# hwwang55/GraphGAN

Hardware: AMD Instinct MI355X
Metric: sampled_edges_per_sec (higher is better)
Workload: dtype f32

## Files before the change

### graphgan_amd/csrc/gg_api.hip

```cpp
#include <stdarg.h>
#include <stdlib.h>
#include <string.h>
#include <sys/stat.h>
#include <unistd.h>

#include <algorithm>
#include <atomic>
#include <thread>

#include "gg_internal.h"

namespace gg {

thread_local std::string g_last_error;

int fail(gg_ctx *ctx, int code, const char *fmt, ...) {
    char buf[1024];
    va_list ap;
    va_start(ap, fmt);
    vsnprintf(buf, sizeof(buf), fmt, ap);
    va_end(ap);
    g_last_error = buf;
    if (ctx) ctx->err = buf;
    return code;
// ... 199 lines not shown
    ctx->w_nslots = n_slots;
    ctx->w_uniform = (!n_walks && uniform_walks >= 0) ? uniform_walks : -1;
    ctx->w_args = {for_d, seed, stream};
    ctx->g_paths_valid = false;
    if (ctx->g_slots_ready) {
        GG_HIP(ctx, hipStreamWaitEvent(ctx->stream, ctx->ev_slots_done, 0));
        ctx->g_slots_ready = false;
        ctx->g_slots_unused++;
    }
    if (n_slots == 0) {
        ctx->walk_stream = ctx->stream;
        return GG_OK;
    }
    return launch_and_join(ctx, n_slots, total, for_d, seed, stream, stride, !defer_join);
}

int gg::walk_finalize(gg_ctx *ctx, bool *retried) {
    if (retried) *retried = false;
    if (ctx->w_nslots == 0) {
        GG_HIP(ctx, hipStreamSynchronize(ctx->stream));
        return GG_OK;
    }
    const int64_t total = ctx->w_total;
    unsigned long long *c = ctx->h_pin;
    constexpr int CW = gg_ctx::CTR_WORDS;
    GG_HIP(ctx, hipMemcpyAsync(c, ctx->dev_ctr, sizeof(unsigned long long) * 2 * CW, hipMemcpyDeviceToHost, ctx->stream));
    GG_HIP(ctx, hipStreamSynchronize(ctx->stream));
    harvest_timings(ctx);
    for (int attempt = 0; c[3] == 2ull || (c[2] != 0ull && ctx->t_lazy); ++attempt) {
        GG_CHECK(ctx, attempt < 16, GG_EHIP, "walk: the launch was voided %d times in a row", attempt);
        if (c[2] != 0ull && ctx->t_lazy) {
            int rebuilt = 0;
            int rc = lazy_fallback_rebuild(ctx, &rebuilt);
            if (rc == GG_ECAPACITY) rc = lazy_rebuild_whole(ctx);
            if (rc != GG_OK) return rc;
            if (ctx->tree_max_depth + 3 > ctx->w_stride) {
                ctx->w_stride = ctx->tree_max_depth + 3;
                GG_HIP(ctx, ctx->w_paths.reserve(sizeof(int32_t) * ((size_t)total * ctx->w_stride + 1)));
            }
        } else {
            ctx->walk_force_sized = true;
        }
        ctx->ctr.walk_reruns += 1;
        generator_changed(ctx);
        int rc = launch_and_join(ctx, ctx->w_nslots, total, ctx->w_args.for_d, ctx->w_args.seed, ctx->w_args.stream, ctx->w_stride);
        ctx->walk_force_sized = false;
        if (rc != GG_OK) return rc;
        GG_HIP(ctx, hipMemcpyAsync(c, ctx->dev_ctr, sizeof(unsigned long long) * 2 * CW, hipMemcpyDeviceToHost, ctx->stream));
        GG_HIP(ctx, hipStreamSynchronize(ctx->stream));
        if (retried) *retried = true;
    }
    const int n_half = ctx->w_split ? 2 : 1;
    if (n_half == 2)
        for (int i = 8; i < CW; ++i) c[i] += c[CW + i];
    {
        int64_t *prof = ctx->alive_prof[ctx->w_args.for_d ? 1 : 0];
        const int run = ctx->w_levels_run;
        for (int i = 0; i < 64; ++i) prof[i] = i < run ? (int64_t)c[8 + i] : -1;
        if (run > 0 && run < 64 && ctx->w_fin_follows) prof[run] = (int64_t)c[7];
        if (ctx->w_net && c[7] > 2048ull && ctx->lv_levels_learned < ctx->tree_max_depth + 2) ctx->lv_levels_learned += 1;
    }
    unsigned long long hops = c[0], reads = c[1], rows = c[5];
    unsigned long long gathers = 0, nodes = 0;
    for (int i = 0; i < 64; ++i) { hops += c[264 + i]; reads += c[328 + i]; rows += c[200 + i]; gathers += c[520 + i]; nodes += c[584 + i]; }
    ctx->ctr.es_gathers += (int64_t)gathers;
    ctx->ctr.es_nodes += (int64_t)nodes;
    ctx->ctr.hops += (int64_t)hops;
    ctx->ctr.nbr_reads += (int64_t)reads;
    ctx->ctr.rows_scored += (int64_t)rows;
    ctx->ctr.walks += total;
    if (total && ctx->walk_timed) {
        float ms = 0.f;
        GG_HIP(ctx, hipEventElapsedTime(&ms, ctx->ev0, ctx->ev1));
        ctx->ctr.last_kernel_ms = ms;
        ctx->ctr.walk_kernel_ms += ms;
        ctx->ctr.walk_launches += 1;
        for (int i = 0; i < ctx->lv_ev_used; ++i) {
            float lms = 0.f;
            for (int k = 0; k < n_half; ++k) {
                float e = 0.f;
                GG_HIP(ctx, hipEventElapsedTime(&e, ctx->lv_ev[4 * i + 2 * k], ctx->lv_ev[4 * i + 2 * k + 1]));
                lms += e;
            }
            ctx->ctr.score_kernel_ms += lms;
            ctx->ctr.score_launches += n_half;
            ctx->ctr.score_chunks += (int64_t)(c[136 + i] >> 32);
            if (getenv("GG_WALK_DEBUG"))
                fprintf(stderr, "[walk] for_d=%d level %d alive %llu score chunks %llu prefix chunks %llu big %llu small %llu rows %llu score %.1f us\n", ctx->w_args.for_d, i,
                        c[8 + i], c[136 + i] >> 32, c[136 + i] & 0xffffffffull, c[72 + i] & 0xffffffffull, c[72 + i] >> 32, c[456 + i], lms * 1e3);
        }
        if (ctx->lv_ev_used) {
            ctx->ctr.score_rows += (int64_t)(rows - c[5]);
            unsigned long long dists = 0;
            for (int i = 0; i < 64; ++i) dists += c[392 + i];
            ctx->ctr.score_dists += (int64_t)dists;
            ctx->ctr.score_gathers += (int64_t)gathers;
            ctx->ctr.score_nodes += (int64_t)nodes;
        }
    }
    if (c[3] || c[6]) generator_changed(ctx);
    if (c[3]) return fail(ctx, GG_ECAPACITY, "walk: a path needed more than stride=%d entries", ctx->w_stride);
    if (c[6]) return fail(ctx, GG_EINVAL, "walk: non-finite generator scores (a softmax had total weight 0, or the generator's tables hold a non-finite value)");
    return GG_OK;
}

int gg::walk_resident(gg_ctx *ctx, const int32_t *slots, const int32_t *n_walks, int32_t uniform_walks, int32_t n_slots,
                      int32_t for_d, uint64_t seed, uint32_t stream, int32_t stride) {
    int rc = walk_launch_async(ctx, slots, n_walks, uniform_walks, n_slots, for_d, seed, stream, stride);
    if (rc != GG_OK) return rc;
    return walk_finalize(ctx, nullptr);
}

extern "C" {

int gg_abi_version(void) { return GG_ABI_VERSION; }

const char *gg_last_error(const gg_ctx *ctx) { return ctx ? ctx->err.c_str() : g_last_error.c_str(); }

int gg_create(int32_t n_node, int32_t n_emb, const float *emb_gen, const float *emb_dis, const gg_config *cfg,
              gg_ctx **out) {
    if (!out) return fail(nullptr, GG_EINVAL, "gg_create: out is NULL");
    *out = nullptr;
    if (n_node <= 0 || n_emb <= 0 || n_emb > 512 || !emb_gen || !emb_dis || !cfg)
        return fail(nullptr, GG_EINVAL, "gg_create: bad argument (n_node=%d n_emb=%d)", n_node, n_emb);
    int ndev = 0;
    hipError_t e = hipGetDeviceCount(&ndev);
    if (e != hipSuccess || ndev <= 0)
        return fail(nullptr, GG_EHIP, "gg_create: no HIP device (%s); this engine has no CPU fallback",
                    e == hipSuccess ? "count = 0" : hipGetErrorString(e));
    if (cfg->device < 0 || cfg->device >= ndev) return fail(nullptr, GG_EINVAL, "gg_create: device %d of %d", cfg->device, ndev);
    hipDeviceProp_t prop;
    GG_HIP(nullptr, hipGetDeviceProperties(&prop, cfg->device));
    if (strncmp(prop.gcnArchName, "gfx950", 6) != 0)
        return fail(nullptr, GG_EHIP, "gg_create: device %d is %s; kernels are built for gfx950 only", cfg->device, prop.gcnArchName);
    GG_HIP(nullptr, hipSetDevice(cfg->device));

    gg_ctx *ctx = new gg_ctx();
    ctx->n_node = n_node;
    ctx->n_emb = n_emb;
    ctx->ld = (n_emb + 3) / 4 * 4;
    ctx->cfg = *cfg;
    ctx->device = cfg->device;
    ctx->n_cus = prop.multiProcessorCount > 0 ? prop.multiProcessorCount : 256;
    if (const char *lv = getenv("GG_WALK_LEVELS")) ctx->walk_levels = atoi(lv);
    if (const char *pe = getenv("GG_PROFILE_EVERY")) ctx->profile_every = std::max(0, atoi(pe));
    if (const char *fw = getenv("GG_COMM_FAKE_WORLD")) ctx->fake_world = atoi(fw);
    if (const char *ow = getenv("GG_COMM_OWNER")) ctx->owner_exchange = atoi(ow);
    if (const char *bf = getenv("GG_COMM_BF16")) ctx->comm_bf16 = atoi(bf) != 0;
    if (const char *om = getenv("GG_COMM_OWNER_MIN")) ctx->owner_min_bound = atoll(om);
    if (const char *dt = getenv("GG_DETERMINISTIC")) ctx->deterministic = atoi(dt) != 0;
    if (const char *nc = getenv("GG_NO_DIST_CACHE")) ctx->dc_enabled = atoi(nc) == 0;
    if (const char *ft = getenv("GG_FIN_THRESHOLD")) ctx->fin_threshold = std::max(0, atoi(ft));
    if (const char *st = getenv("GG_STAGE_T")) ctx->sg_threshold = std::max(0, atoi(st));
    if (const char *ws = getenv("GG_WALK_SPLIT")) ctx->split_enabled = atoi(ws) != 0;
    if (const char *em = getenv("GG_ES_MODE")) ctx->es_mode = std::min(2, std::max(0, atoi(em)));
    if (const char *er = getenv("GG_ES_RATIO")) ctx->es_ratio_num = std::max(1, atoi(er));
    if (const char *eh = getenv("GG_ES_HUB")) ctx->es_hub = std::max(0, atoi(eh));
    if (const char *wm = getenv("GG_WALK_SPLIT_MIN")) ctx->split_min_walks = std::max(512, atoi(wm));
    for (auto &m : ctx->alive_prof) for (auto &v : m) v = -1;
    if (const char *dr = getenv("GG_COMM_DENSE_RATIO")) ctx->dense_exchange_ratio = (float)atof(dr);
#define GG_TRY(call)                        \
    do {                                    \
        int rc__ = (call);                  \
        if (rc__ != GG_OK) {                \
            g_last_error = ctx->err;        \
            gg_destroy(ctx);                \
            return rc__;                    \
        }                                   \
    } while (0)
    auto body = [&]() -> int {
        GG_HIP(ctx, hipStreamCreateWithFlags(&ctx->stream, hipStreamNonBlocking));
        {
            int lo = 0, hi = 0;
            const char *wp = getenv("GG_WALK_PRIORITY");
            if (wp && atoi(wp) != 0 && hipDeviceGetStreamPriorityRange(&lo, &hi) == hipSuccess && hi != lo)
                GG_HIP(ctx, hipStreamCreateWithPriority(&ctx->stream2, hipStreamNonBlocking, atoi(wp) > 0 ? hi : lo));
            else
                GG_HIP(ctx, hipStreamCreateWithFlags(&ctx->stream2, hipStreamNonBlocking));
        }
        GG_HIP(ctx, hipStreamCreateWithFlags(&ctx->stream3, hipStreamNonBlocking));
        GG_HIP(ctx, hipEventCreateWithFlags(&ctx->ev_fork, hipEventDisableTiming));
        GG_HIP(ctx, hipEventCreateWithFlags(&ctx->ev_join, hipEventDisableTiming));
        GG_HIP(ctx, hipEventCreateWithFlags(&ctx->ev_score[0], hipEventDisableTiming));
        GG_HIP(ctx, hipEventCreateWithFlags(&ctx->ev_score[1], hipEventDisableTiming));
        ctx->walk_stream = ctx->stream;
        GG_HIP(ctx, hipEventCreate(&ctx->ev0));
        GG_HIP(ctx, hipEventCreate(&ctx->ev1));
        GG_HIP(ctx, hipEventCreateWithFlags(&ctx->ev_walk_done, hipEventDisableTiming));
        GG_HIP(ctx, hipEventCreateWithFlags(&ctx->ev_gen_pass, hipEventDisableTiming));
        GG_HIP(ctx, hipEventCreateWithFlags(&ctx->ev_main_mark, hipEventDisableTiming));
        GG_HIP(ctx, hipHostMalloc((void **)&ctx->h_pin, sizeof(unsigned long long) * gg_ctx::PIN_WORDS, hipHostMallocDefault));
        memset(ctx->h_pin, 0, sizeof(unsigned long long) * gg_ctx::PIN_WORDS);
        const size_t tb = sizeof(float) * (size_t)n_node * ctx->ld, vb = sizeof(float) * (size_t)n_node;
        for (int m = 0; m < 2; ++m) {
            Model &M = ctx->model[m];
            GG_HIP(ctx, hipMalloc((void **)&M.E, tb));
            GG_HIP(ctx, hipMalloc((void **)&M.b, vb));
            GG_HIP(ctx, hipMemset(M.b, 0, vb));
            if (cfg->optimizer != GG_OPT_SGD) {
                GG_HIP(ctx, hipMalloc((void **)&M.mE, tb));
                GG_HIP(ctx, hipMalloc((void **)&M.vE, tb));
                GG_HIP(ctx, hipMalloc((void **)&M.mb, vb));
                GG_HIP(ctx, hipMalloc((void **)&M.vb, vb));
                GG_HIP(ctx, hipMemset(M.mE, 0, tb));
                GG_HIP(ctx, hipMemset(M.vE, 0, tb));
                GG_HIP(ctx, hipMemset(M.mb, 0, vb));
                GG_HIP(ctx, hipMemset(M.vb, 0, vb));
            }
            M.b1p = cfg->adam_beta1;
            M.b2p = cfg->adam_beta2;
            M.lr = m == 0 ? cfg->lr_gen : cfg->lr_dis;
            M.lambda = m == 0 ? cfg->lambda_gen : cfg->lambda_dis;
            int rc = upload_table(ctx, M.E, m == 0 ? emb_gen : emb_dis);
            if (rc != GG_OK) return rc;
        }
        GG_HIP(ctx, hipMalloc((void **)&ctx->gradE, tb));
        GG_HIP(ctx, hipMalloc((void **)&ctx->gradb, vb));
        GG_HIP(ctx, hipMemset(ctx->gradE, 0, tb));
        ctx->grad_elems_padded = (size_t)n_node * ctx->ld;
        GG_HIP(ctx, hipMemset(ctx->gradb, 0, vb));
        GG_HIP(ctx, hipMalloc((void **)&ctx->touched, sizeof(int32_t) * n_node));
        GG_HIP(ctx, hipMalloc((void **)&ctx->touched_list, sizeof(int32_t) * n_node));
        GG_HIP(ctx, hipMalloc((void **)&ctx->touched_cnt, sizeof(int32_t) * 4));
        GG_HIP(ctx, hipMemset(ctx->touched, 0, sizeof(int32_t) * n_node));
        GG_HIP(ctx, hipMemset(ctx->touched_cnt, 0, sizeof(int32_t) * 4));
        GG_HIP(ctx, hipMalloc((void **)&ctx->dev_ctr, sizeof(unsigned long long) * gg_ctx::PIN_WORDS));
        GG_HIP(ctx, hipMemset(ctx->dev_ctr, 0, sizeof(unsigned long long) * gg_ctx::PIN_WORDS));
        GG_HIP(ctx, ctx->table_bad.reserve(sizeof(unsigned long long) * 2));
        for (int m = 0; m < 2; ++m) {
            int rc = rescan_table_finite(ctx, m);
            if (rc != GG_OK) return rc;
        }
        GG_HIP(ctx, hipDeviceSynchronize());
        return GG_OK;
    };
    GG_TRY(body());
#undef GG_TRY
    *out = ctx;
    return GG_OK;
}

int gg_destroy(gg_ctx *ctx) {
    if (!ctx) return GG_OK;
    (void)hipSetDevice(ctx->device);
    if (ctx->stream) (void)hipStreamSynchronize(ctx->stream);
    if (ctx->stream2) (void)hipStreamSynchronize(ctx->stream2);
    comm_destroy(ctx);
    for (int m = 0; m < 2; ++m) {
        Model &M = ctx->model[m];
        float *ps[] = {M.E, M.b, M.mE, M.vE, M.mb, M.vb};
        for (float *p : ps)
            if (p) (void)hipFree(p);
    }
    void *ps[] = {ctx->gradE, ctx->gradb, ctx->touched, ctx->touched_list, ctx->touched_cnt, ctx->g_rowptr, ctx->g_col, ctx->dev_ctr,
                  ctx->es, ctx->es_stamp, ctx->g_rev};
    for (void *p : ps)
        if (p) (void)hipFree(p);
    free_trees(ctx);
    DevBuf *bufs[] = {&ctx->w_slots_m[0], &ctx->w_slots_m[1], &ctx->w_ptr_m[0], &ctx->w_ptr_m[1], &ctx->w_samples, &ctx->w_paths, &ctx->w_len, &ctx->w_status,
                      &ctx->w_first, &ctx->w_abort, &ctx->w_scratch, &ctx->d_center, &ctx->d_neighbor, &ctx->d_label, &ctx->d_cnt,
                      &ctx->d_ptr, &ctx->g_node1, &ctx->g_node2, &ctx->g_reward, &ctx->g_cnt, &ctx->g_ptr, &ctx->scan_tmp,
                      &ctx->step_u, &ctx->step_v, &ctx->step_x, &ctx->sg_cnt, &ctx->sg_off, &ctx->sg_slot, &ctx->sg_list, &ctx->sg_rows, &ctx->sg_bias, &ctx->sg_tot, &ctx->sg_key, &ctx->touched_ptr, &ctx->x_cnt, &ctx->x_send_ids, &ctx->x_send_rows,
                      &ctx->x_recv_ids, &ctx->x_recv_rows, &ctx->x_nglob, &ctx->x_own, &ctx->st_item, &ctx->st_item2, &ctx->st_cur, &ctx->st_prev, &ctx->st_len,
                      &ctx->st_alive, &ctx->st_rank, &ctx->bfs_key, &ctx->bfs_bm, &ctx->bfs_misc, &ctx->bfs_sparse, &ctx->bfs_rowptr32, &ctx->lv_pfx, &ctx->dc_keys, &ctx->dc_vals, &ctx->dc_words, &ctx->lv_beg, &ctx->lv_k, &ctx->lv_chunks, &ctx->lv_coff, &ctx->lv_scores, &ctx->lv_chunk_owner, &ctx->lv_prefix, &ctx->lv_big, &ctx->lv_fe, &ctx->fin_list, &ctx->table_bad, &ctx->sgp_cnt, &ctx->sgp_off, &ctx->sgp_slot, &ctx->sgp_list, &ctx->sgp_tot, &ctx->sgp_key, &ctx->sgp_scan, &ctx->sgp_hub, &ctx->sg_hub, &ctx->hub_acc,
                      &ctx->q3_store, &ctx->q3s_off, &ctx->ep_center, &ctx->ep_neighbor, &ctx->ep_label, &ctx->ep_node1, &ctx->ep_node2, &ctx->ep_reward, &ctx->topk_adj,
                      &ctx->gs_es, &ctx->gs_cpre, &ctx->pt_starts, &ctx->pt_paths, &ctx->pt_len, &ctx->pt_cnt, &ctx->pt_ptr, &ctx->pt_noise, &ctx->pt_sample};
    for (DevBuf *b : bufs) b->release();
    for (hipEvent_t e : ctx->lv_ev)
        if (e) (void)hipEventDestroy(e);
    for (auto &tr : ctx->tm_ev)
        for (hipEvent_t e : tr)
            if (e) (void)hipEventDestroy(e);
    for (hipEvent_t e : ctx->pt_ev)
        if (e) (void)hipEventDestroy(e);
    if (ctx->h_pin) (void)hipHostFree(ctx->h_pin);
    for (hipEvent_t e : {ctx->ev_walk_done, ctx->ev_slots_done, ctx->ev_gen_pass, ctx->ev_main_mark, ctx->ev_fork, ctx->ev_join, ctx->ev_score[0], ctx->ev_score[1]})
        if (e) (void)hipEventDestroy(e);
    if (ctx->stream3) {
        (void)hipStreamSynchronize(ctx->stream3);
        (void)hipStreamDestroy(ctx->stream3);
    }
    if (ctx->stream2) {
        (void)hipStreamSynchronize(ctx->stream2);
        (void)hipStreamDestroy(ctx->stream2);
    }
    if (ctx->ev0) (void)hipEventDestroy(ctx->ev0);
    if (ctx->ev1) (void)hipEventDestroy(ctx->ev1);
    if (ctx->stream) (void)hipStreamDestroy(ctx->stream);
    delete ctx;
    return GG_OK;
}

int gg_set_graph_csr(gg_ctx *ctx, const int64_t *rowptr, const int32_t *col) {
    if (!ctx) return fail(nullptr, GG_EINVAL, "ctx is NULL");
    GG_CHECK(ctx, rowptr && rowptr[0] == 0, GG_EINVAL, "gg_set_graph_csr: rowptr[0] must be 0");
    discard_begun_walk(ctx);
    const int n = ctx->n_node;
    const int64_t nnz = rowptr[n];
    GG_CHECK(ctx, nnz >= 0 && (col || nnz == 0), GG_EINVAL, "gg_set_graph_csr: col is NULL");
    for (int v = 0; v < n; ++v) GG_CHECK(ctx, rowptr[v + 1] >= rowptr[v], GG_EINVAL, "gg_set_graph_csr: rowptr not monotone at %d", v);
    for (int64_t e = 0; e < nnz; ++e) GG_CHECK(ctx, col[e] >= 0 && col[e] < n, GG_EINVAL, "gg_set_graph_csr: col[%lld]=%d out of range", (long long)e, col[e]);
    GG_HIP(ctx, hipSetDevice(ctx->device));
    (void)hipDeviceSynchronize();
    for (void *p : {(void *)ctx->g_rowptr, (void *)ctx->g_col, (void *)ctx->es, (void *)ctx->es_stamp, (void *)ctx->g_rev})
        if (p) (void)hipFree(p);
    ctx->g_rowptr = nullptr;
// ... 652 lines not shown
```

### graphgan_amd/csrc/gg_internal.h

```cpp
#pragma once
#include <hip/hip_runtime.h>
#include <stdint.h>
#include <stdio.h>
#include <string>
#include <vector>

#include "../../include/graphgan_hip.h"

namespace gg {

struct DevBuf {
    void *p = nullptr;
    size_t bytes = 0;
    hipError_t reserve(size_t need) {
        if (need <= bytes) return hipSuccess;
        if (p) {
            (void)hipDeviceSynchronize();
            (void)hipFree(p);
        }
        p = nullptr;
        bytes = 0;
        size_t want = need + need / 4 + 256;
        hipError_t e = hipMalloc(&p, want);
        if (e == hipSuccess) bytes = want;
// ... 17 lines not shown
};

}

struct gg_ctx {
    int32_t n_node = 0, n_emb = 0, ld = 0;
    gg_config cfg{};
    int device = 0;
    hipStream_t stream = nullptr;
    hipEvent_t ev0 = nullptr, ev1 = nullptr;
    hipStream_t stream2 = nullptr;
    hipStream_t walk_stream = nullptr;
    hipEvent_t ev_walk_done = nullptr;
    hipEvent_t ev_gen_pass = nullptr;
    hipEvent_t ev_main_mark = nullptr;
    bool gen_pass_recorded = false;
    bool gen_dirty = false;
    hipEvent_t lv_ev[256] = {};
    hipStream_t stream3 = nullptr;
    hipEvent_t ev_fork = nullptr, ev_join = nullptr, ev_score[2] = {nullptr, nullptr};
    bool split_enabled = false;
    int64_t split_min_walks = 32768;
    bool w_split = false;
    gg::DevBuf fin_list;
    gg::DevBuf table_bad;
    int lv_ev_used = 0;
    gg::Model model[2];

    float *gradE = nullptr, *gradb = nullptr;
    int32_t *touched = nullptr;
    int32_t *touched_list = nullptr;
    int32_t *touched_cnt = nullptr;

    int64_t *g_rowptr = nullptr;
    int32_t *g_col = nullptr;
    int64_t g_nnz = 0;
    uint64_t g_hash = 0;
    std::vector<int64_t> h_rowptr;
    std::vector<int32_t> h_col;
    float *es = nullptr;
    long long *es_stamp = nullptr;
    int32_t *g_rev = nullptr;
    long long es_tick = 256;
    long long es_valid_from = 256;
    int32_t es_mode = 1;
    int32_t es_ratio_num = 2;
    int32_t es_hub = 0;

    int32_t n_tree_roots = 0, tree_max_depth = 0, tree_max_list = 0;
    int64_t tree_nodes = 0;
    int64_t t_cap_nodes = 0, t_cap_roots = 0, t_cap_q3 = 0;
    int64_t tree_entries = 0;
    int32_t *t_root = nullptr;
    int32_t *t_order = nullptr;
    int32_t *t_cstart = nullptr;
    int32_t *t_edge = nullptr;
    bool t_edge_valid = false;
    int64_t *t_base = nullptr;
    uint32_t *t_q3 = nullptr;
    int64_t *t_q3off = nullptr;
    std::vector<int32_t> h_troot;
    std::vector<int64_t> h_tbase, h_q3off;
    std::vector<int32_t> h_comp_size;

    int32_t tree_mode = -1;
    int64_t lz_cap = 0;
    bool t_lazy = false;
    bool lz_force_whole = false;
    int32_t lz_min_level = 0x7fffffff;
    uint32_t lz_stamp = 0;
    gg::DevBuf lz_info, lz_pair, lz_rank, lz_bm, lz_cursor, lz_flag, lz_limit, lz_expect, lz_list, lz_scratch, lz_fb_scratch;
    int64_t arena_next = 0, arena_end = 0;
    int64_t lz_fallback_roots = 0, lz_fallback_rounds = 0, lz_resolved = 0;
    bool g_multi = true;
    int32_t g_max_deg = 0;

    gg::DevBuf w_slots_m[2], w_ptr_m[2];
    std::vector<int32_t> h_slots_m[2];
    std::vector<int64_t> h_ptr_m[2], h_ptr_new;
    int w_mode = 0;
    int64_t alive_prof[2][64];
    int64_t fin_threshold = 0;
    int w_levels_run = 0;
    bool w_fin_follows = false;
    bool w_net = false;
    const gg::DevBuf &w_slots_buf() const { return w_slots_m[w_mode]; }
    const gg::DevBuf &w_ptr_buf() const { return w_ptr_m[w_mode]; }
    gg::DevBuf w_samples, w_paths, w_len, w_status, w_first, w_abort, w_scratch;
    gg::DevBuf st_cur, st_prev, st_len, st_alive, st_rank, st_item, st_item2, lv_beg, lv_k, lv_chunks, lv_coff, lv_scores, lv_chunk_owner, lv_prefix, lv_big, lv_fe;
    gg::DevBuf lv_pfx, dc_keys, dc_vals, dc_words;
    size_t dc_size = 0;
    int32_t dc_request = 0;
    bool dc_valid = false;
    bool dc_enabled = true;
    int64_t lv_cap_total = 0;
    int32_t lv_levels_learned = 0;
    int64_t lv_cap_chunks = 0;
    bool walk_force_sized = false;
    bool walk_used_speculation = false;
    int32_t walk_levels = 64;
    int64_t w_total = 0;
    int32_t w_stride = 0, w_nslots = 0;
    int32_t w_uniform = -1;
    struct { int32_t for_d; uint64_t seed; uint32_t stream; } w_args{};

    static constexpr int CTR_WORDS = 720;
    static constexpr int PIN_WORDS = 2048;
    static constexpr int H_TOTAL = 1960;
    static constexpr int H_ROWS = 1940;
    unsigned long long *h_pin = nullptr;
    int32_t profile_every = 1;
    int64_t walk_call_index = 0;
    bool walk_timed = false;
    bool profile_solo = true;
    struct PendingTiming { int kind; int64_t units; int slot; bool has_rows; };
    hipEvent_t tm_ev[8][3] = {};
    std::vector<PendingTiming> tm_pending;
    int64_t pass_call_index[2] = {0, 0};
    int tm_cur = -1;

    gg::DevBuf d_center, d_neighbor, d_label, d_cnt, d_ptr;
    int64_t d_rows = 0;
    gg::DevBuf g_node1, g_node2, g_reward, g_cnt, g_ptr;
    int64_t g_pairs = 0;
    bool g_paths_valid = false;
    bool g_begun = false;
    struct { int32_t n_slots = 0, n_sample = 0; uint64_t seed = 0; uint32_t stream = 0; } g_begun_args;
    gg::DevBuf touched_ptr;
    gg::DevBuf bfs_key, bfs_bm, bfs_misc, bfs_sparse, bfs_rowptr32;
    bool bfs_rowptr32_valid = false;
    gg::DevBuf q3_store, q3s_off;
    int64_t q3_words = 0;
    bool q3_store_ready = false;
    gg::DevBuf ep_center, ep_neighbor, ep_label, ep_node1, ep_node2, ep_reward;
    int64_t ep_rows = 0, ep_pairs = 0;
    std::vector<int32_t> ep_slots;
    bool in_epoch_add = false;
    int n_cus = 256;
    gg::DevBuf scan_tmp, step_u, step_v, step_x;
    gg::DevBuf sg_cnt, sg_off, sg_slot, sg_list, sg_rows, sg_bias, sg_tot, sg_key;
    bool g_pairs_filled = false;
    bool sg_cnt_dirty = false;
    gg::DevBuf sgp_cnt, sgp_off, sgp_slot, sgp_list, sgp_tot, sgp_key, sgp_scan, sgp_hub;
    gg::DevBuf sg_hub, hub_acc;
    int64_t hub_cap = 0;
    hipEvent_t ev_slots_done = nullptr;
    bool g_slots_ready = false;
    bool sgp_cnt_clean = false;
    int g_slots_unused = 0;
    int64_t g_slots_walks = 0;
    int32_t g_slots_stride = 0;
    int32_t *sg_cnt_active = nullptr;
    bool sg_active = false;
    int sg_threshold = 64;

    unsigned long long *dev_ctr = nullptr;
    gg_counters ctr{};

    void *comm = nullptr;
    bool comm_rsag = true;
    size_t grad_elems_padded = 0;
    int64_t d_rows_max = 0, g_pairs_max = 0;
    int64_t step_bound = 0;
    int64_t comm_steps_sparse = 0, comm_steps_dense = 0, comm_bytes_sent = 0;
    int32_t rank = 0, world = 1;
    bool deterministic = true;
    float dense_exchange_ratio = 1.5f;
    int32_t fake_world = 0;
    gg::DevBuf x_cnt, x_send_ids, x_send_rows, x_recv_ids, x_recv_rows;
    gg::DevBuf x_nglob;
    gg::DevBuf x_own;
    int32_t owner_exchange = 1;
    bool comm_bf16 = false;
    int64_t owner_min_bound = 4096;
    int64_t comm_steps_owner = 0;

    gg::DevBuf topk_adj;
    bool topk_adj_valid = false;

    gg::DevBuf gs_es, gs_cpre;
    int64_t gs_chunks = 0;
    bool gs_es_valid = false, gs_cpre_valid = false;

    gg::DevBuf pt_starts, pt_paths, pt_len, pt_cnt, pt_ptr, pt_noise, pt_sample;
    bool pt_noise_set = false;
    uint64_t pt_noise_total = 0;
    int32_t pt_sample_n = 0, pt_sample_stride = 1;
    hipEvent_t pt_ev[4] = {};
    bool ep_d_open = false;

    std::string err;
};

namespace gg {

extern thread_local std::string g_last_error;

int fail(gg_ctx *ctx, int code, const char *fmt, ...);

#define GG_HIP(ctx, call)                                                                      \
    do {                                                                                       \
        hipError_t e__ = (call);                                                               \
        if (e__ != hipSuccess)                                                                 \
            return gg::fail(ctx, GG_EHIP, "%s:%d %s -> %s", __FILE__, __LINE__, #call,         \
                            hipGetErrorString(e__));                                           \
    } while (0)

#define GG_CHECK(ctx, cond, code, ...)                        \
    do {                                                      \
        if (!(cond)) return gg::fail(ctx, code, __VA_ARGS__); \
    } while (0)

int device_exclusive_scan(gg_ctx *ctx, const int32_t *cnt, int64_t *ptr, int64_t n);
int ensure_g_pairs(gg_ctx *ctx);
int device_compact_flags(gg_ctx *ctx, const int32_t *flag, int64_t n, int32_t *list, int64_t *total_out);
int device_segment_rows(gg_ctx *ctx, const int32_t *cnt, int64_t n, int T, int32_t *off, int4 *list, int64_t *totals, hipStream_t stream = nullptr,
                        DevBuf *scratch = nullptr);

int alloc_trees(gg_ctx *ctx, const int32_t *roots, int32_t n_roots, const int64_t *node_counts, const int64_t *root_children, int64_t extra_nodes = 0);
bool lazy_build_wanted(const gg_ctx *ctx);
int lazy_rebuild_whole(gg_ctx *ctx);
int lazy_fallback_rebuild(gg_ctx *ctx, int *n_out);
void component_sizes(int n, const int64_t *rowptr, const int32_t *col, std::vector<int32_t> &comp_size);
int32_t host_bfs_order(const int64_t *rowptr, const int32_t *col, int32_t root, int32_t *order, int32_t *cstart,
                       std::vector<uint32_t> &stamp, uint32_t &epoch, int32_t *depth_out, int32_t *max_children_out);
void order_to_lists(int32_t n, int32_t C, const int32_t *order, const int32_t *cstart, const uint32_t *q3, int32_t *off, int32_t *nbr);
int32_t lists_to_order(int32_t n, int32_t root, const int32_t *off, const int32_t *nbr, int32_t *order, int32_t *cstart,
                       uint32_t *q3, int32_t q3_words, int32_t *depth_out, int32_t *max_children_out);

int walk_launch_async(gg_ctx *ctx, const int32_t *slots, const int32_t *n_walks, int32_t uniform_walks, int32_t n_slots,
                      int32_t for_d, uint64_t seed, uint32_t stream, int32_t stride, bool side_stream = false, bool defer_join = false);
void discard_begun_walk(gg_ctx *ctx);
int walk_finalize(gg_ctx *ctx, bool *retried);
int timing_slot(gg_ctx *ctx);
int check_exchange_flag(gg_ctx *ctx);
void harvest_timings(gg_ctx *ctx);
int derive_tree_edges(gg_ctx *ctx);
int compute_reverse_edges(gg_ctx *ctx);
int rescan_table_finite(gg_ctx *ctx, int which);
int enqueue_path_slots(gg_ctx *ctx);
void generator_changed(gg_ctx *ctx);
int walk_resident(gg_ctx *ctx, const int32_t *slots, const int32_t *n_walks, int32_t uniform_walks, int32_t n_slots,
                  int32_t for_d, uint64_t seed, uint32_t stream, int32_t stride);
int launch_walk_sample(gg_ctx *ctx, int32_t n_slots, int64_t total_walks, int for_d, uint64_t seed, uint32_t stream,
                       int32_t stride);
int run_step(gg_ctx *ctx, int which, const int32_t *d_u, const int32_t *d_v, const float *d_x, int32_t n);
int comm_allreduce_grads(gg_ctx *ctx);
int comm_allreduce_flags(gg_ctx *ctx);
int comm_allreduce_i64(gg_ctx *ctx, int64_t *buf, size_t count);
int comm_allreduce_max_i64(gg_ctx *ctx, int64_t *buf, size_t count);
size_t comm_dense_bytes(const gg_ctx *ctx);
int exchange_count_max(gg_ctx *ctx, int64_t local, int64_t *max_out);
int comm_allgather(gg_ctx *ctx, const void *send, void *recv, size_t count, int elem_bytes);
bool comm_has_p2p(const gg_ctx *ctx);
int comm_exchange_v(gg_ctx *ctx, const float *send, const int64_t *send_off, const int64_t *send_cnt, float *recv, const int64_t *recv_off,
                    const int64_t *recv_cnt);
void comm_destroy(gg_ctx *ctx);

static inline int cdiv(int64_t a, int64_t b) { return (int)((a + b - 1) / b); }

}
```

### graphgan_amd/csrc/prepare.hip

```cpp
#include <algorithm>

#include <cstring>

#include "gg_internal.h"

namespace gg {

constexpr int SCAN_THREADS = 256;
constexpr int SCAN_ITEMS = 8;
constexpr int SCAN_TILE = SCAN_THREADS * SCAN_ITEMS;

__device__ __forceinline__ int64_t block_excl_scan(int64_t v, int64_t *total, int64_t *sh ) {
    const int lane = threadIdx.x & 63, wv = threadIdx.x >> 6;
    int64_t inc = v;
#pragma unroll
    for (int off = 1; off < 64; off <<= 1) {
        const int64_t o = __shfl_up(inc, off, 64);
        if (lane >= off) inc += o;
    }
    if (lane == 63) sh[wv] = inc;
    __syncthreads();
    int64_t base = 0, tot = 0;
#pragma unroll
    for (int i = 0; i < SCAN_THREADS / 64; ++i) {
        if (i < wv) base += sh[i];
        tot += sh[i];
    }
    __syncthreads();
    *total = tot;
    return base + inc - v;
}

__global__ __launch_bounds__(SCAN_THREADS) void scan_tile_sums(const int32_t *cnt, int64_t n, int64_t *tile_sum) {
    __shared__ int64_t sh[SCAN_THREADS / 64];
    const int64_t base = (int64_t)blockIdx.x * SCAN_TILE + (int64_t)threadIdx.x * SCAN_ITEMS;
    int64_t s = 0;
#pragma unroll
    for (int i = 0; i < SCAN_ITEMS; ++i)
        if (base + i < n) s += cnt[base + i];
    int64_t tot;
    (void)block_excl_scan(s, &tot, sh);
    if (threadIdx.x == 0) tile_sum[blockIdx.x] = tot;
}

__global__ __launch_bounds__(SCAN_THREADS) void scan_tile_offsets(int64_t *tile_sum, int64_t n_tiles, int64_t *total_out) {
    __shared__ int64_t sh[SCAN_THREADS / 64];
    int64_t carry = 0;
    for (int64_t t0 = 0; t0 < n_tiles; t0 += SCAN_THREADS) {
        const int64_t i = t0 + threadIdx.x;
        const int64_t v = i < n_tiles ? tile_sum[i] : 0;
        int64_t tot;
        const int64_t ex = block_excl_scan(v, &tot, sh);
        if (i < n_tiles) tile_sum[i] = carry + ex;
        carry += tot;
    }
    if (threadIdx.x == 0) *total_out = carry;
}

__global__ __launch_bounds__(SCAN_THREADS) void scan_tile_offsets2(int64_t *tile_sum_a, int64_t *tile_sum_b, int64_t n_tiles, int64_t *total_a, int64_t *total_b) {
    __shared__ int64_t sh[SCAN_THREADS / 64];
    int64_t *const tile_sum = blockIdx.x == 0 ? tile_sum_a : tile_sum_b;
    int64_t carry = 0;
    for (int64_t t0 = 0; t0 < n_tiles; t0 += SCAN_THREADS) {
        const int64_t i = t0 + threadIdx.x;
        const int64_t v = i < n_tiles ? tile_sum[i] : 0;
        int64_t tot;
        const int64_t ex = block_excl_scan(v, &tot, sh);
        if (i < n_tiles) tile_sum[i] = carry + ex;
        carry += tot;
    }
    if (threadIdx.x == 0) *(blockIdx.x == 0 ? total_a : total_b) = carry;
}

__global__ __launch_bounds__(SCAN_THREADS) void scan_apply(const int32_t *cnt, int64_t n, const int64_t *tile_off, int64_t *ptr) {
    __shared__ int64_t sh[SCAN_THREADS / 64];
    const int64_t base = (int64_t)blockIdx.x * SCAN_TILE + (int64_t)threadIdx.x * SCAN_ITEMS;
    int64_t v[SCAN_ITEMS], s = 0;
#pragma unroll
    for (int i = 0; i < SCAN_ITEMS; ++i) {
        v[i] = base + i < n ? cnt[base + i] : 0;
        s += v[i];
    }
    int64_t tot;
    int64_t run = tile_off[blockIdx.x] + block_excl_scan(s, &tot, sh);
#pragma unroll
    for (int i = 0; i < SCAN_ITEMS; ++i) {
        if (base + i < n) ptr[base + i] = run;
        run += v[i];
    }
}

int device_exclusive_scan(gg_ctx *ctx, const int32_t *cnt, int64_t *ptr, int64_t n) {
    const int64_t tiles = (n + SCAN_TILE - 1) / SCAN_TILE;
    GG_HIP(ctx, ctx->scan_tmp.reserve(sizeof(int64_t) * (tiles + 2)));
    int64_t *ts = ctx->scan_tmp.as<int64_t>();
    if (n == 0) {
        GG_HIP(ctx, hipMemsetAsync(ptr, 0, sizeof(int64_t), ctx->stream));
        return GG_OK;
    }
    hipLaunchKernelGGL(scan_tile_sums, dim3((unsigned)tiles), dim3(SCAN_THREADS), 0, ctx->stream, cnt, n, ts);
    hipLaunchKernelGGL(scan_tile_offsets, dim3(1), dim3(SCAN_THREADS), 0, ctx->stream, ts, tiles, ptr + n);
    hipLaunchKernelGGL(scan_apply, dim3((unsigned)tiles), dim3(SCAN_THREADS), 0, ctx->stream, cnt, n, ts, ptr);
    GG_HIP(ctx, hipGetLastError());
    return GG_OK;
}

__global__ __launch_bounds__(SCAN_THREADS) void flag_tile_sums(const int32_t *flag, int64_t n, int64_t *tile_sum) {
    __shared__ int64_t sh[SCAN_THREADS / 64];
    const int64_t base = (int64_t)blockIdx.x * SCAN_TILE + (int64_t)threadIdx.x * SCAN_ITEMS;
    int64_t s = 0;
#pragma unroll
    for (int i = 0; i < SCAN_ITEMS; ++i)
        if (base + i < n) s += flag[base + i] > 0 ? 1 : 0;
    int64_t tot;
    (void)block_excl_scan(s, &tot, sh);
    if (threadIdx.x == 0) tile_sum[blockIdx.x] = tot;
}

__global__ __launch_bounds__(SCAN_THREADS) void flag_compact(const int32_t *flag, int64_t n, const int64_t *tile_off, int32_t *list) {
    __shared__ int64_t sh[SCAN_THREADS / 64];
    const int64_t base = (int64_t)blockIdx.x * SCAN_TILE + (int64_t)threadIdx.x * SCAN_ITEMS;
    bool v[SCAN_ITEMS];
    int64_t s = 0;
#pragma unroll
    for (int i = 0; i < SCAN_ITEMS; ++i) {
        v[i] = base + i < n && flag[base + i] > 0;
        s += v[i] ? 1 : 0;
    }
    int64_t tot;
    int64_t run = tile_off[blockIdx.x] + block_excl_scan(s, &tot, sh);
#pragma unroll
    for (int i = 0; i < SCAN_ITEMS; ++i)
        if (v[i]) list[run++] = (int32_t)(base + i);
}

int device_compact_flags(gg_ctx *ctx, const int32_t *flag, int64_t n, int32_t *list, int64_t *total_out) {
    const int64_t tiles = (n + SCAN_TILE - 1) / SCAN_TILE;
    GG_HIP(ctx, ctx->scan_tmp.reserve(sizeof(int64_t) * (tiles + 2)));
    int64_t *ts = ctx->scan_tmp.as<int64_t>();
    if (n == 0) {
        GG_HIP(ctx, hipMemsetAsync(total_out, 0, sizeof(int64_t), ctx->stream));
        return GG_OK;
    }
    hipLaunchKernelGGL(flag_tile_sums, dim3((unsigned)tiles), dim3(SCAN_THREADS), 0, ctx->stream, flag, n, ts);
    hipLaunchKernelGGL(scan_tile_offsets, dim3(1), dim3(SCAN_THREADS), 0, ctx->stream, ts, tiles, total_out);
    hipLaunchKernelGGL(flag_compact, dim3((unsigned)tiles), dim3(SCAN_THREADS), 0, ctx->stream, flag, n, ts, list);
    GG_HIP(ctx, hipGetLastError());
    return GG_OK;
}

__global__ __launch_bounds__(SCAN_THREADS) void seg_tile_sums(const int32_t *cnt, int64_t n, int T, int64_t *tile_rows, int64_t *tile_occ) {
    __shared__ int64_t sh[SCAN_THREADS / 64];
    const int64_t base = (int64_t)blockIdx.x * SCAN_TILE + (int64_t)threadIdx.x * SCAN_ITEMS;
    int64_t rows = 0, occ = 0;
#pragma unroll
    for (int i = 0; i < SCAN_ITEMS; ++i)
        if (base + i < n) {
            const int c = cnt[base + i];
            if (c > 0 && c <= T) { rows += 1; occ += c; }
        }
    int64_t tot;
    (void)block_excl_scan(rows, &tot, sh);
    if (threadIdx.x == 0) tile_rows[blockIdx.x] = tot;
    (void)block_excl_scan(occ, &tot, sh);
    if (threadIdx.x == 0) tile_occ[blockIdx.x] = tot;
}

__global__ __launch_bounds__(SCAN_THREADS) void seg_apply(const int32_t *cnt, int64_t n, int T, const int64_t *tile_rows, const int64_t *tile_occ,
                                                          int32_t *off, int4 *list) {
    __shared__ int64_t sh[SCAN_THREADS / 64];
    const int64_t base = (int64_t)blockIdx.x * SCAN_TILE + (int64_t)threadIdx.x * SCAN_ITEMS;
    int c[SCAN_ITEMS];
    int64_t rows = 0, occ = 0;
#pragma unroll
    for (int i = 0; i < SCAN_ITEMS; ++i) {
        const int v = base + i < n ? cnt[base + i] : 0;
        c[i] = (v > 0 && v <= T) ? v : 0;
        rows += c[i] ? 1 : 0;
        occ += c[i];
    }
    int64_t tot;
    int64_t rrun = tile_rows[blockIdx.x] + block_excl_scan(rows, &tot, sh);
    int64_t orun = tile_occ[blockIdx.x] + block_excl_scan(occ, &tot, sh);
#pragma unroll
    for (int i = 0; i < SCAN_ITEMS; ++i)
        if (c[i]) {
            list[rrun++] = make_int4((int32_t)(base + i), (int32_t)orun, c[i], 0);
            off[base + i] = (int32_t)orun;
            orun += c[i];
        }
}

int device_segment_rows(gg_ctx *ctx, const int32_t *cnt, int64_t n, int T, int32_t *off, int4 *list, int64_t *totals, hipStream_t stream, DevBuf *scratch) {
    const int64_t tiles = (n + SCAN_TILE - 1) / SCAN_TILE;
    if (!scratch) scratch = &ctx->scan_tmp;
    if (!stream) stream = ctx->stream;
    GG_HIP(ctx, scratch->reserve(sizeof(int64_t) * (2 * tiles + 4)));
    int64_t *tr = scratch->as<int64_t>(), *to = tr + tiles + 1;
    hipLaunchKernelGGL(seg_tile_sums, dim3((unsigned)tiles), dim3(SCAN_THREADS), 0, stream, cnt, n, T, tr, to);
    hipLaunchKernelGGL(scan_tile_offsets2, dim3(2), dim3(SCAN_THREADS), 0, stream, tr, to, tiles, totals, totals + 1);
    hipLaunchKernelGGL(seg_apply, dim3((unsigned)tiles), dim3(SCAN_THREADS), 0, stream, cnt, n, T, tr, to, off, list);
    GG_HIP(ctx, hipGetLastError());
    return GG_OK;
}

__global__ void pair_count_kernel(const int32_t *path_len, int64_t n_walks, int window, int32_t *cnt, const unsigned long long *flag) {
    const int64_t w = (int64_t)blockIdx.x * blockDim.x + threadIdx.x;
    if (w >= n_walks) return;
    if (*flag == 2ull) { cnt[w] = 0; return; }
    const int L = path_len[w] - 1;
    int c = 0;
    for (int i = 0; i < L; ++i) {
        const int lo = max(i - window, 0), hi = min(i + window + 1, L);
        c += hi - lo - 1;
    }
    cnt[w] = L > 0 ? c : 0;
}

__global__ void pair_fill_kernel(const int32_t *paths, const int32_t *path_len, int stride, int64_t n_walks, int window,
                                 const int64_t *ptr, int32_t *node1, int32_t *node2, const unsigned long long *flag) {
    const int64_t w = (int64_t)blockIdx.x * blockDim.x + threadIdx.x;
    if (w >= n_walks || *flag == 2ull) return;
    const int L = path_len[w] - 1;
    const int32_t *p = paths + w * (int64_t)stride;
    int64_t o = ptr[w];
    for (int i = 0; i < L; ++i) {
        const int lo = max(i - window, 0), hi = min(i + window + 1, L);
        const int c = p[i];
        for (int j = lo; j < hi; ++j) {
            if (j == i) continue;
            node1[o] = c;
            node2[o] = p[j];
            ++o;
        }
    }
}

__global__ __launch_bounds__(256) void pair_reward_kernel(const float *E, const float *bias, int ld, const int32_t *u,
                                                          const int32_t *v, int64_t n_host, const int64_t *n_dev, float *out) {
    const int64_t n = n_dev ? *n_dev : n_host;
    const int t = threadIdx.x & 15;
    const int64_t g0 = ((int64_t)blockIdx.x * blockDim.x + threadIdx.x) >> 4;
    const int64_t ng = ((int64_t)gridDim.x * blockDim.x) >> 4;
    const int nchunk = ld >> 2;
    for (int64_t p = g0; p < n; p += ng) {
        const int a = u[p], b = v[p];
        const float4 *ra = (const float4 *)(E + (int64_t)a * ld);
        const float4 *rb = (const float4 *)(E + (int64_t)b * ld);
        float acc = 0.f;
        for (int c = t; c < nchunk; c += 16) {
            const float4 x = ra[c], y = rb[c];
            acc = __builtin_fmaf(x.x, y.x, acc);
            acc = __builtin_fmaf(x.y, y.y, acc);
            acc = __builtin_fmaf(x.z, y.z, acc);
            acc = __builtin_fmaf(x.w, y.w, acc);
        }
        acc += __shfl_xor(acc, 8, 64);
        acc += __shfl_xor(acc, 4, 64);
        acc += __shfl_xor(acc, 2, 64);
        acc += __shfl_xor(acc, 1, 64);
        if (t == 0) {
            float s = acc + bias[b];
            s = fminf(fmaxf(s, -10.0f), 10.0f);
            out[p] = logf(1.0f + expf(s));
        }
    }
}

template <int NCH>
__global__ __launch_bounds__(256) void path_reward_kernel(const float *E, const float *bias, int ld, const int32_t *paths,
                                                          const int32_t *path_len, int stride, int64_t n_walks, int window,
                                                          const int64_t *ptr, float *out, const unsigned long long *flag) {
    const int t = threadIdx.x & 15;
    const int64_t w = ((int64_t)blockIdx.x * blockDim.x + threadIdx.x) >> 4;
    if (w >= n_walks || *flag == 2ull) return;
    const int L = path_len[w] - 1;
    if (L <= 1) return;
    const int32_t *p = paths + w * (int64_t)stride;
    const int nchunk = ld >> 2;
    const int64_t pi0 = ptr[w];
    float4 R[3][NCH];
    float bv[3];
    bool have[3];
    auto fetch = [&](int pos, float4 (&row)[NCH], float &b, bool &ok) {
        ok = pos >= 0 && pos < L;
        const int nd = ok ? p[pos] : 0;
        b = ok ? bias[nd] : 0.f;
        const float4 *r = (const float4 *)(E + (int64_t)nd * ld);
#pragma unroll
        for (int i = 0; i < NCH; ++i) {
            const int c = t + 16 * i;
            row[i] = (ok && c < nchunk) ? r[c] : make_float4(0.f, 0.f, 0.f, 0.f);
        }
    };
    fetch(0, R[0], bv[0], have[0]);
    fetch(1, R[1], bv[1], have[1]);
    fetch(2, R[2], bv[2], have[2]);
    auto n_pairs_of = [&](int i) { return min(i, window) + min(L - 1 - i, window); };
    int base = 0;
    for (int c = 0; c < L; ++c) {
        float4 Rn[NCH];
        float nb;
        bool nh;
        fetch(c + 3, Rn, nb, nh);
        const int back_c = min(c, window);
        int base_d = base + n_pairs_of(c);
        float myval = 0.f;
        int myidx = -1;
#pragma unroll
        for (int d = 1; d <= 2; ++d) {
            if (d <= window && have[d]) {
                float acc = 0.f;
#pragma unroll
                for (int i = 0; i < NCH; ++i) {
                    acc = __builtin_fmaf(R[0][i].x, R[d][i].x, acc);
                    acc = __builtin_fmaf(R[0][i].y, R[d][i].y, acc);
                    acc = __builtin_fmaf(R[0][i].z, R[d][i].z, acc);
                    acc = __builtin_fmaf(R[0][i].w, R[d][i].w, acc);
                }
                acc += __shfl_xor(acc, 8, 64);
                acc += __shfl_xor(acc, 4, 64);
                acc += __shfl_xor(acc, 2, 64);
                acc += __shfl_xor(acc, 1, 64);
                if (t == 2 * d - 2) { myval = acc + bv[d]; myidx = base + back_c + (d - 1); }
                if (t == 2 * d - 1) { myval = acc + bv[0]; myidx = base_d + (c - max(c + d - window, 0)); }
            }
            base_d += n_pairs_of(c + d);
        }
        if (myidx >= 0) {
            const float sc = fminf(fmaxf(myval, -10.0f), 10.0f);
            out[pi0 + myidx] = logf(1.0f + expf(sc));
        }
        base += n_pairs_of(c);
#pragma unroll
        for (int i = 0; i < NCH; ++i) { R[0][i] = R[1][i]; R[1][i] = R[2][i]; R[2][i] = Rn[i]; }
        have[0] = have[1]; have[1] = have[2]; have[2] = nh;
        bv[0] = bv[1]; bv[1] = bv[2]; bv[2] = nb;
    }
}

__global__ __launch_bounds__(256) void edge_dot_f64_kernel(const float *E, int ld, const int32_t *u, const int32_t *v, int64_t n, double *out) {
    const int t = threadIdx.x & 15;
    const int64_t g0 = ((int64_t)blockIdx.x * blockDim.x + threadIdx.x) >> 4, ng = ((int64_t)gridDim.x * blockDim.x) >> 4;
    for (int64_t p = g0; p < n; p += ng) {
        const float *ra = E + (int64_t)u[p] * ld, *rb = E + (int64_t)v[p] * ld;
        double acc = 0.0;
        for (int k = t; k < ld; k += 16) acc = fma((double)ra[k], (double)rb[k], acc);
        acc += __shfl_xor(acc, 8, 64);
        acc += __shfl_xor(acc, 4, 64);
        acc += __shfl_xor(acc, 2, 64);
        acc += __shfl_xor(acc, 1, 64);
        if (t == 0) out[p] = acc;
    }
}
// ... 315 lines not shown
```

### graphgan_amd/csrc/steps.hip

```cpp
#include <stdlib.h>

#include <algorithm>
#include <cmath>
#include <vector>

#include "gg_internal.h"

namespace gg {

struct HubAcc {
    unsigned long long *acc;
    int64_t cap;
    float scale;
};
__device__ __forceinline__ unsigned long long *hub_row(const HubAcc &h, int slot, int ld) {
    const int64_t k = -3 - (int64_t)slot;
    return (slot <= -3 && k < h.cap) ? h.acc + k * (ld + 1) : nullptr;
}
__device__ __forceinline__ void hub_add(unsigned long long *p, float x, float scale) {
    atomicAdd(p, (unsigned long long)__float2ll_rn(x * scale));
}

struct StepArgs {
    float *E, *b;
    float *gE, *gb;
    int32_t *touched, *touched_list, *touched_cnt;
    int ld, track;
    const int32_t *u, *v;
    const float *x;
    int n;
    float lambda, inv_n;
    const int64_t *n_glob;
    int is_d;
    int ppg;
    unsigned long long *prof;
    const int32_t *slot_v, *slot_u;
    float *stage, *stage_b;
    HubAcc hub;
};

__global__ __launch_bounds__(256) void pair_occ_count_kernel(const int32_t *u, const int32_t *v, int n, int ppg, int32_t *cnt,
                                                             int32_t *slot_v, int32_t *slot_u) {
    const int p = blockIdx.x * blockDim.x + threadIdx.x;
    if (p >= n) return;
    slot_v[p] = atomicAdd(&cnt[v[p]], 1);
    const bool run_end = p == n - 1 || (p + 1) % ppg == 0 || u[p + 1] != u[p];
    slot_u[p] = run_end ? atomicAdd(&cnt[u[p]], 1) : -2;
}

__global__ __launch_bounds__(256) void pair_occ_slot_kernel(const int32_t *u, const int32_t *v, int n, const int32_t *cnt, const int32_t *off,
                                                            int T, int32_t *slot_v, int32_t *slot_u, int32_t *key) {
    const int p = blockIdx.x * blockDim.x + threadIdx.x;
    if (p >= n) return;
    const int iv = v[p], iu = u[p];
    const int sv = cnt[iv] <= T ? off[iv] + slot_v[p] : -3 - off[iv];
    slot_v[p] = sv;
    if (sv >= 0) key[sv] = 2 * p + 1;
    if (slot_u[p] != -2) {
        const int su = cnt[iu] <= T ? off[iu] + slot_u[p] : -3 - off[iu];
        slot_u[p] = su;
        if (su >= 0) key[su] = 2 * p;
    }
}

constexpr int PAIRS_PER_GROUP = 16;

template <int NF, bool STAGED>
__global__ __launch_bounds__(256) void pair_grad_kernel(const StepArgs a) {
    const int t = threadIdx.x & 15;
    const int g = (blockIdx.x * blockDim.x + threadIdx.x) >> 4;
    const int p0 = g * a.ppg;
    if (p0 >= a.n) return;
    const int p1 = min(p0 + a.ppg, a.n);
    const int nchunk = a.ld >> 2;
    const float inv_n = a.n_glob ? 1.0f / (float)(*a.n_glob) : a.inv_n;
    float accu[NF];
#pragma unroll
    for (int i = 0; i < NF; ++i) accu[i] = 0.f;
    int run_u = a.u[p0];
    auto flush_u = [&](int q) {
        const int sl = STAGED ? a.slot_u[q] : -1;
        if (STAGED && sl >= 0) {
            float *g = a.stage + (int64_t)sl * a.ld;
#pragma unroll
            for (int i = 0; i < NF; ++i) {
                const int f = t + 16 * i;
                if (f < a.ld) g[f] = accu[i];
            }
            if (t == 0) a.stage_b[sl] = 0.f;
            return;
        }
        float *gu = a.gE + (int64_t)run_u * a.ld;
#pragma unroll
        for (int i = 0; i < NF; ++i) {
            const int f = t + 16 * i;
            if (f < a.ld) atomicAdd(gu + f, accu[i]);
        }
        if (t == 0 && a.track) a.touched[run_u] = 1;
    };
    for (int p = p0; p < p1; ++p) {
        const int iu = a.u[p], iv = a.v[p];
        if (iu != run_u) {
            flush_u(p - 1);
#pragma unroll
            for (int i = 0; i < NF; ++i) accu[i] = 0.f;
            run_u = iu;
        }
        const float4 *ru = (const float4 *)(a.E + (int64_t)iu * a.ld);
        const float4 *rv = (const float4 *)(a.E + (int64_t)iv * a.ld);
        float acc = 0.f;
        for (int c = t; c < nchunk; c += 16) {
            const float4 x = ru[c], y = rv[c];
            acc = __builtin_fmaf(x.x, y.x, acc);
            acc = __builtin_fmaf(x.y, y.y, acc);
            acc = __builtin_fmaf(x.z, y.z, acc);
            acc = __builtin_fmaf(x.w, y.w, acc);
        }
        acc += __shfl_xor(acc, 8, 64);
        acc += __shfl_xor(acc, 4, 64);
        acc += __shfl_xor(acc, 2, 64);
        acc += __shfl_xor(acc, 1, 64);
        const float bv = a.b[iv];
        const float s = acc + bv;
        const float sg = 1.0f / (1.0f + expf(-s));
        float ds;
        if (a.is_d) {
            ds = sg - a.x[p];
        } else {
            const bool inside = (sg >= 1e-5f) && (sg <= 1.0f);
            ds = inside ? -(a.x[p] * inv_n) * (1.0f - sg) : 0.0f;
        }
        const float *fu = (const float *)ru, *fv = (const float *)rv;
        const int slv = STAGED ? a.slot_v[p] : -1;
        const bool st = STAGED && slv >= 0;
        float *gv = st ? a.stage + (int64_t)slv * a.ld : a.gE + (int64_t)iv * a.ld;
#pragma unroll
        for (int i = 0; i < NF; ++i) {
            const int f = t + 16 * i;
            if (f < a.ld) {
                const float x = fu[f], y = fv[f];
                accu[i] += ds * y + a.lambda * x;
                const float gval = ds * x + a.lambda * y;
                if (st) gv[f] = gval;
                else atomicAdd(gv + f, gval);
            }
        }
        if (t == 0) {
            const float gbv = a.is_d ? ds + a.lambda * bv : ds;
            if (st) {
                a.stage_b[slv] = gbv;
            } else {
                atomicAdd(a.gb + iv, gbv);
                if (a.track) a.touched[iv] = 1;
            }
        }
    }
    flush_u(p1 - 1);
}

template <int NF, bool STAGED>
__global__ __launch_bounds__(256) void pair_grad16_kernel(const StepArgs a) {
    const int t = threadIdx.x & 15;
    const int64_t g = ((int64_t)blockIdx.x * blockDim.x + threadIdx.x) >> 4;
    const int64_t p0 = g * 16;
    if (p0 >= a.n) return;
    const int np = (int)min((int64_t)16, (int64_t)a.n - p0);
    const float inv_n = a.n_glob ? 1.0f / (float)(*a.n_glob) : a.inv_n;
    const bool mine = t < np;
    const int myu = mine ? a.u[p0 + t] : 0, myv = mine ? a.v[p0 + t] : 0;
    const float myx = mine ? a.x[p0 + t] : 0.f;
    const int my_sv = (STAGED && mine) ? a.slot_v[p0 + t] : -1;
    const int my_su = (STAGED && mine) ? a.slot_u[p0 + t] : -1;
    const float mybv = a.b[myv];
    const int nextu = __shfl(myu, (t + 1) & 15, 16);
    const bool my_end = mine && (t == np - 1 || nextu != myu);
    auto fetch = [&](int j, float (&ru)[NF], float (&rv)[NF]) {
        const int jj = j < np ? j : 0;
        const float *su = a.E + (int64_t)__shfl(myu, jj, 16) * a.ld, *sv = a.E + (int64_t)__shfl(myv, jj, 16) * a.ld;
#pragma unroll
        for (int i = 0; i < NF; ++i) {
            const int f = t + 16 * i;
            const int fc = f < a.ld ? f : a.ld - 1;
            ru[i] = su[fc];
            rv[i] = sv[fc];
        }
    };
    float U[3][NF], V[3][NF], accu[NF];
#pragma unroll
    for (int i = 0; i < NF; ++i) accu[i] = 0.f;
    fetch(0, U[0], V[0]);
    fetch(1, U[1], V[1]);
#pragma unroll 1
    for (int j0 = 0; j0 < np; j0 += 3) {
#pragma unroll
        for (int r = 0; r < 3; ++r) {
            const int j = j0 + r;
            if (j >= np) break;
            fetch(j + 2, U[(r + 2) % 3], V[(r + 2) % 3]);
            float acc = 0.f;
#pragma unroll
            for (int i = 0; i < NF; ++i) {
                const bool in = t + 16 * i < a.ld;
                const float x = in ? U[r][i] : 0.f, y = in ? V[r][i] : 0.f;
                U[r][i] = x; V[r][i] = y;
                acc = __builtin_fmaf(x, y, acc);
            }
            acc += __shfl_xor(acc, 8, 64);
            acc += __shfl_xor(acc, 4, 64);
            acc += __shfl_xor(acc, 2, 64);
            acc += __shfl_xor(acc, 1, 64);
            const float bv = __shfl(mybv, j, 16), xj = __shfl(myx, j, 16);
            const float s = acc + bv;
            const float sg = 1.0f / (1.0f + expf(-s));
            float ds;
            if (a.is_d) {
                ds = sg - xj;
            } else {
                const bool inside = (sg >= 1e-5f) && (sg <= 1.0f);
                ds = inside ? -(xj * inv_n) * (1.0f - sg) : 0.0f;
            }
            const int iv = __shfl(myv, j, 16), iu = __shfl(myu, j, 16);
            const int slv = __shfl(my_sv, j, 16), slu = __shfl(my_su, j, 16);
            const bool st = STAGED && slv >= 0;
            unsigned long long *hv = STAGED && !st ? hub_row(a.hub, slv, a.ld) : nullptr;
            float *gv = st ? a.stage + (int64_t)slv * a.ld : a.gE + (int64_t)iv * a.ld;
#pragma unroll
            for (int i = 0; i < NF; ++i) {
                const int f = t + 16 * i;
                if (f < a.ld) {
                    accu[i] += ds * V[r][i] + a.lambda * U[r][i];
                    const float gval = ds * U[r][i] + a.lambda * V[r][i];
                    if (st) gv[f] = gval;
                    else if (STAGED && hv) hub_add(hv + f, gval, a.hub.scale);
                    else atomicAdd(gv + f, gval);
                }
            }
            if (t == 0) {
                const float gbv = a.is_d ? ds + a.lambda * bv : ds;
                if (st) {
                    a.stage_b[slv] = gbv;
                } else {
                    if (STAGED && hv) hub_add(hv + a.ld, gbv, a.hub.scale);
                    else atomicAdd(a.gb + iv, gbv);
                    if (a.track) a.touched[iv] = 1;
                }
            }
            if (__shfl((int)my_end, j, 16)) {
                if (STAGED && slu >= 0) {
                    float *gu = a.stage + (int64_t)slu * a.ld;
#pragma unroll
                    for (int i = 0; i < NF; ++i) {
                        const int f = t + 16 * i;
                        if (f < a.ld) gu[f] = accu[i];
                    }
                    if (t == 0) a.stage_b[slu] = 0.f;
                } else {
                    float *gu = a.gE + (int64_t)iu * a.ld;
                    unsigned long long *hu = STAGED ? hub_row(a.hub, slu, a.ld) : nullptr;
#pragma unroll
                    for (int i = 0; i < NF; ++i) {
                        const int f = t + 16 * i;
                        if (f < a.ld) {
                            if (STAGED && hu) hub_add(hu + f, accu[i], a.hub.scale);
                            else atomicAdd(gu + f, accu[i]);
                        }
                    }
                    if (t == 0 && a.track) a.touched[iu] = 1;
                }
#pragma unroll
                for (int i = 0; i < NF; ++i) accu[i] = 0.f;
            }
        }
    }
}

struct PathArgs {
    float *E, *b, *gE, *gb;
    int32_t *touched, *touched_list, *touched_cnt;
    int ld, track, window;
    const int32_t *paths, *path_len;
    int stride;
    const int64_t *pair_ptr;
    const float *reward;
    int64_t n_walks;
    float lambda, inv_n;
    const int64_t *n_glob;
    const int32_t *slot;
    float *stage, *stage_b;
    HubAcc hub;
};

__global__ __launch_bounds__(256) void path_count_kernel(const int32_t *paths, const int32_t *path_len, int stride, int64_t n_walks,
                                                         int32_t *cnt, int32_t *slot, const unsigned long long *flag) {
    const int64_t idx = (int64_t)blockIdx.x * blockDim.x + threadIdx.x;
    const int64_t w = idx / stride;
    if (w >= n_walks || (flag && *flag == 2ull)) return;
    const int c = (int)(idx - w * stride), L = path_len[w] - 1;
    if (L <= 1 || c >= L) return;
    slot[idx] = atomicAdd(&cnt[paths[idx]], 1);
}

__global__ __launch_bounds__(256) void path_slot_kernel(const int32_t *paths, const int32_t *path_len, int stride, int64_t n_walks,
                                                        const int32_t *cnt, const int32_t *off, int T, int32_t *slot, int32_t *key, const unsigned long long *flag) {
    const int64_t idx = (int64_t)blockIdx.x * blockDim.x + threadIdx.x;
    const int64_t w = idx / stride;
    if (w >= n_walks || (flag && *flag == 2ull)) return;
    const int c = (int)(idx - w * stride), L = path_len[w] - 1;
    if (L <= 1 || c >= L) return;
    const int nd = paths[idx];
    const int sl = cnt[nd] <= T ? off[nd] + slot[idx] : -3 - off[nd];
    slot[idx] = sl;
    if (sl >= 0) key[sl] = (int32_t)idx;
}

template <int NF, bool STAGED, bool SHORT>
__global__ __launch_bounds__(256) __attribute__((amdgpu_waves_per_eu(NF <= 8 ? 3 : 1, 4))) void path_grad_kernel(const PathArgs a) {
    const int t = threadIdx.x & 15;
    const int64_t w = ((int64_t)blockIdx.x * blockDim.x + threadIdx.x) >> 4;
    if (w >= a.n_walks) return;
    const int L = a.path_len[w] - 1;
    if (L <= 1) return;
    const float inv_n = a.n_glob ? 1.0f / (float)(*a.n_glob) : a.inv_n;
    const int32_t *p = a.paths + w * (int64_t)a.stride;
    int64_t pi = a.pair_ptr[w];
    const int32_t *const wslot = STAGED ? a.slot + w * (int64_t)a.stride : nullptr;
    const int myid = (t < L) ? p[t] : -1;
    const int myslot = (STAGED && t < L) ? wslot[t] : -1;
    const int64_t pi0 = pi;
    const int n_pairs = (int)(a.pair_ptr[w + 1] - pi0);
    float rwl[4];
#pragma unroll
    for (int q = 0; q < 4; ++q) rwl[q] = (16 * q + t < n_pairs) ? a.reward[pi0 + 16 * q + t] : 0.f;
    auto id_at = [&](int pos) -> int {
        if (SHORT) {
            const int v = __shfl(myid, pos & 15, 16);
            return (pos >= 0 && pos < L) ? v : -1;
        }
        return (pos >= 0 && pos < L) ? (pos < 16 ? __shfl(myid, pos, 16) : p[pos]) : -1;
    };
    auto slot_at = [&](int pos) -> int {
        if (!STAGED) return -1;
        if (SHORT) {
            const int v = __shfl(myslot, pos & 15, 16);
            return (pos >= 0 && pos < L) ? v : -1;
        }
        return (pos >= 0 && pos < L) ? (pos < 16 ? __shfl(myslot, pos, 16) : wslot[pos]) : -1;
    };
    auto reward_at = [&](int k, int64_t pidx) -> float {
        const float v0 = __shfl(rwl[0], k & 15, 16), v1 = __shfl(rwl[1], k & 15, 16);
        const float v2 = __shfl(rwl[2], k & 15, 16), v3 = __shfl(rwl[3], k & 15, 16);
        const float v = k < 16 ? v0 : (k < 32 ? v1 : (k < 48 ? v2 : v3));
        if (SHORT) return v;
        return k < 64 ? v : a.reward[pidx];
    };
    float R[3][NF], A[3][NF], bv[3], gb[3], npair[3];
    int node[3], sslot[3];
#pragma unroll
    for (int sl = 0; sl < 3; ++sl) {
        node[sl] = -1; bv[sl] = 0.f; gb[sl] = 0.f; sslot[sl] = -1; npair[sl] = 0.f;
#pragma unroll
        for (int i = 0; i < NF; ++i) { R[sl][i] = 0.f; A[sl][i] = 0.f; }
    }
    auto fetch_raw = [&](int pos, float (&row)[NF], int &nd_out, int &slot_out, float &b_out) {
        const int nd = id_at(pos);
        const int ndc = nd >= 0 ? nd : 0;
        b_out = a.b[ndc];
        const float *src = a.E + (int64_t)ndc * a.ld;
#pragma unroll
        for (int i = 0; i < NF; ++i) {
            const int f = t + 16 * i;
            row[i] = src[f < a.ld ? f : a.ld - 1];
        }
        nd_out = nd;
        slot_out = slot_at(pos);
    };
    auto enter = [&](int sl, const float (&row)[NF], int nd, int slot, float b) {
        node[sl] = nd; sslot[sl] = slot; gb[sl] = 0.f; npair[sl] = 0.f;
        bv[sl] = nd >= 0 ? b : 0.f;
#pragma unroll
        for (int i = 0; i < NF; ++i) {
            R[sl][i] = (nd >= 0 && t + 16 * i < a.ld) ? row[i] : 0.f;
            A[sl][i] = 0.f;
        }
    };
    auto flush = [&](int sl) {
        const int nd = node[sl];
        if (nd < 0) return;
        const float lam_n = a.lambda * npair[sl];
#pragma unroll
        for (int i = 0; i < NF; ++i) A[sl][i] = __builtin_fmaf(lam_n, R[sl][i], A[sl][i]);
        if (STAGED && sslot[sl] >= 0) {
            float *g = a.stage + (int64_t)sslot[sl] * a.ld;
#pragma unroll
            for (int i = 0; i < NF; ++i) {
                const int f = t + 16 * i;
                if (f < a.ld) g[f] = A[sl][i];
            }
            if (t == 0) a.stage_b[sslot[sl]] = gb[sl];
            return;
        }
        float *g = a.gE + (int64_t)nd * a.ld;
        unsigned long long *h = STAGED ? hub_row(a.hub, sslot[sl], a.ld) : nullptr;
#pragma unroll
        for (int i = 0; i < NF; ++i) {
            const int f = t + 16 * i;
            if (f < a.ld) {
                if (STAGED && h) hub_add(h + f, A[sl][i], a.hub.scale);
                else atomicAdd(g + f, A[sl][i]);
            }
        }
        if (t == 0) {
            if (STAGED && h) {
                if (gb[sl] != 0.f) hub_add(h + a.ld, gb[sl], a.hub.scale);
            } else if (gb[sl] != 0.f) {
                atomicAdd(a.gb + nd, gb[sl]);
            }
            if (a.track) a.touched[nd] = 1;
        }
    };
    float Rq[2][NF], qbv[2];
    int qnode[2], qslot[2];
    {
        float r0[NF], r1[NF], r2[NF], b0, b1, b2;
        int n0, n1, n2, s0, s1, s2;
        fetch_raw(0, r0, n0, s0, b0);
        fetch_raw(1, r1, n1, s1, b1);
        fetch_raw(2, r2, n2, s2, b2);
        fetch_raw(3, Rq[0], qnode[0], qslot[0], qbv[0]);
        enter(0, r0, n0, s0, b0);
        enter(1, r1, n1, s1, b1);
        enter(2, r2, n2, s2, b2);
    }
    auto n_pairs_of = [&](int i) { return min(i, a.window) + min(L - 1 - i, a.window); };
    int base = 0;
    for (int c = 0; c < L; ++c) {
        fetch_raw(c + 4, Rq[1], qnode[1], qslot[1], qbv[1]);
        const int back_c = min(c, a.window);
        int base_d = base + n_pairs_of(c);
        float mys = 0.f;
        int myk = -1;
#pragma unroll
        for (int d = 1; d <= 2; ++d) {
            if (d <= a.window && node[d] >= 0) {
                float acc = 0.f;
#pragma unroll
                for (int i = 0; i < NF; ++i) acc = __builtin_fmaf(R[0][i], R[d][i], acc);
                acc += __shfl_xor(acc, 8, 64);
                acc += __shfl_xor(acc, 4, 64);
                acc += __shfl_xor(acc, 2, 64);
                acc += __shfl_xor(acc, 1, 64);
                if (t == 2 * d - 2) { mys = acc + bv[d]; myk = base + back_c + (d - 1); }
                if (t == 2 * d - 1) { mys = acc + bv[0]; myk = base_d + (c - max(c + d - a.window, 0)); }
            }
            base_d += n_pairs_of(c + d);
        }
        const int kk = myk >= 0 ? myk : 0;
        const float rw = reward_at(kk, pi0 + kk);
        float myds = 0.f;
        if (myk >= 0) {
            const float sg = 1.0f / (1.0f + expf(-mys));
            const bool inside = (sg >= 1e-5f) && (sg <= 1.0f);
            myds = inside ? -(rw * inv_n) * (1.0f - sg) : 0.0f;
        }
#pragma unroll
        for (int d = 1; d <= 2; ++d) {
            const float ds_f = __shfl(myds, 2 * d - 2, 16), ds_r = __shfl(myds, 2 * d - 1, 16);
            if (d <= a.window && node[d] >= 0) {
                const float dsum = ds_f + ds_r;
#pragma unroll
                for (int i = 0; i < NF; ++i) {
                    A[0][i] = __builtin_fmaf(dsum, R[d][i], A[0][i]);
                    A[d][i] = __builtin_fmaf(dsum, R[0][i], A[d][i]);
                }
                npair[0] += 2.0f;
                npair[d] += 2.0f;
                gb[d] += ds_f;
                gb[0] += ds_r;
            }
        }
        base += n_pairs_of(c);
        flush(0);
#pragma unroll
        for (int sl = 0; sl < 2; ++sl) {
            node[sl] = node[sl + 1]; bv[sl] = bv[sl + 1]; gb[sl] = gb[sl + 1]; sslot[sl] = sslot[sl + 1]; npair[sl] = npair[sl + 1];
#pragma unroll
            for (int i = 0; i < NF; ++i) { R[sl][i] = R[sl + 1][i]; A[sl][i] = A[sl + 1][i]; }
        }
        enter(2, Rq[0], qnode[0], qslot[0], qbv[0]);
        qnode[0] = qnode[1]; qbv[0] = qbv[1]; qslot[0] = qslot[1];
#pragma unroll
        for (int i = 0; i < NF; ++i) Rq[0][i] = Rq[1][i];
    }
}

struct OptArgs {
    float *E, *b, *mE, *vE, *mb, *vb, *gE, *gb;
    const int64_t *touched_ptr;
    const int64_t *touched_total;
    int64_t nE;
    int n_node, ld;
    float lr_t, b1, b2, eps, lr;
    int32_t *touched, *touched_list, *touched_cnt;
    int32_t *sg_cnt;
    const int4 *sg_list;
    const int64_t *sg_tot;
    const float *stage, *stage_b;
    const int32_t *stage_key;
    unsigned long long *bad;
};

__device__ __forceinline__ bool nonfinite4(const float4 &x) { return !(__builtin_isfinite(x.x) && __builtin_isfinite(x.y) && __builtin_isfinite(x.z) && __builtin_isfinite(x.w)); }

__device__ __forceinline__ void adam_elem(float &var, float &m, float &v, float g, const OptArgs &a) {
    m = m * a.b1;
    m = m + (1.0f - a.b1) * g;
    v = v * a.b2;
    v = v + (g * g) * (1.0f - a.b2);
    var = var - (a.lr_t * m) / (sqrtf(v) + a.eps);
}

__global__ __launch_bounds__(256) void adam_dense_kernel(const OptArgs a) {
    const int64_t n4 = a.nE >> 2;
    const int64_t stride = (int64_t)gridDim.x * blockDim.x;
    const float4 z = make_float4(0.f, 0.f, 0.f, 0.f);
    bool bad = false;
    for (int64_t i = (int64_t)blockIdx.x * blockDim.x + threadIdx.x; i < n4; i += stride) {
        float4 var = ((float4 *)a.E)[i], m = ((float4 *)a.mE)[i], v = ((float4 *)a.vE)[i];
        const float4 g = ((const float4 *)a.gE)[i];
        adam_elem(var.x, m.x, v.x, g.x, a);
        adam_elem(var.y, m.y, v.y, g.y, a);
        adam_elem(var.z, m.z, v.z, g.z, a);
        adam_elem(var.w, m.w, v.w, g.w, a);
        bad |= nonfinite4(var);
        ((float4 *)a.E)[i] = var;
        ((float4 *)a.mE)[i] = m;
        ((float4 *)a.vE)[i] = v;
        if (g.x != 0.f || g.y != 0.f || g.z != 0.f || g.w != 0.f) ((float4 *)a.gE)[i] = z;
    }
    for (int64_t i = (int64_t)blockIdx.x * blockDim.x + threadIdx.x; i < a.n_node; i += stride) {
        float var = a.b[i], m = a.mb[i], v = a.vb[i];
        const float g = a.gb[i];
        adam_elem(var, m, v, g, a);
        bad |= !__builtin_isfinite(var);
        a.b[i] = var;
        a.mb[i] = m;
        a.vb[i] = v;
        if (g != 0.f) a.gb[i] = 0.f;
    }
    if (bad) *a.bad = 1ull;
}

template <int SGD>
__device__ __forceinline__ void opt_row(const OptArgs &a, int row, int t, int nchunk) {
    const float4 z = make_float4(0.f, 0.f, 0.f, 0.f);
    {
        const int64_t o = ((int64_t)row * a.ld) >> 2;
        for (int c = t; c < nchunk; c += 16) {
            float4 var = ((float4 *)a.E)[o + c];
            const float4 g = ((const float4 *)a.gE)[o + c];
            if (SGD) {
                var.x -= a.lr * g.x; var.y -= a.lr * g.y; var.z -= a.lr * g.z; var.w -= a.lr * g.w;
            } else {
                float4 m = ((float4 *)a.mE)[o + c], v = ((float4 *)a.vE)[o + c];
                adam_elem(var.x, m.x, v.x, g.x, a);
                adam_elem(var.y, m.y, v.y, g.y, a);
                adam_elem(var.z, m.z, v.z, g.z, a);
                adam_elem(var.w, m.w, v.w, g.w, a);
                ((float4 *)a.mE)[o + c] = m;
                ((float4 *)a.vE)[o + c] = v;
            }
            if (nonfinite4(var)) *a.bad = 1ull;
            ((float4 *)a.E)[o + c] = var;
            ((float4 *)a.gE)[o + c] = z;
        }
        if (t == 0) {
            float var = a.b[row];
            const float g = a.gb[row];
            if (SGD) {
                var -= a.lr * g;
            } else {
                float m = a.mb[row], v = a.vb[row];
                adam_elem(var, m, v, g, a);
                a.mb[row] = m;
                a.vb[row] = v;
            }
            if (!__builtin_isfinite(var)) *a.bad = 1ull;
            a.b[row] = var;
            a.gb[row] = 0.f;
            a.touched[row] = 0;
            if (a.sg_cnt) a.sg_cnt[row] = 0;
        }
    }
}

constexpr int DET_MAX_PAIRS = 256;
constexpr int DET_THREADS = 1024;
constexpr int DET_GROUPS = DET_THREADS / 16;
constexpr size_t DET_LDS_ROW_BYTES = 144 * 1024;

__device__ __forceinline__ unsigned group16_ballot(bool pred) {
    const uint64_t m = __ballot(pred);
    return (unsigned)(m >> (threadIdx.x & 48)) & 0xffffu;
}

template <int NF, bool ROWS_IN_LDS, int OPT, bool SMALLN>
__global__ __launch_bounds__(DET_THREADS) void pair_grad_det_kernel(const StepArgs a, const OptArgs o) {
    static_assert(OPT == 0 || ROWS_IN_LDS, "the fused update needs every table read in front of the barrier");
    extern __shared__ float det_rows[];
    __shared__ int32_t ids[2 * DET_MAX_PAIRS];
    __shared__ float coef[DET_MAX_PAIRS], coefb[DET_MAX_PAIRS];
    const int t = threadIdx.x & 15, g = threadIdx.x >> 4;
    const int n = a.n, ld = a.ld, nchunk = ld >> 2;
    const float inv_n = a.n_glob ? 1.0f / (float)(*a.n_glob) : a.inv_n;
    const bool stamp = a.prof && blockIdx.x == 0 && (threadIdx.x == 0 || threadIdx.x == DET_THREADS - 64);
    unsigned long long *const pw = a.prof + (threadIdx.x ? 8 : 0);
    if (stamp) pw[0] = wall_clock64();
    for (int s = threadIdx.x; s < 2 * n; s += DET_THREADS) ids[s] = s < n ? a.u[s] : a.v[s - n];
    for (int p = g; p < n; p += DET_GROUPS) {
        const int iu = a.u[p], iv = a.v[p];
        const float xp = a.x[p];
        const float bv = a.b[iv];
        const float4 *ru = (const float4 *)(a.E + (int64_t)iu * ld);
        const float4 *rv = (const float4 *)(a.E + (int64_t)iv * ld);
        float acc = 0.f;
        for (int c = t; c < nchunk; c += 16) {
            const float4 x = ru[c], y = rv[c];
            if (ROWS_IN_LDS) {
                ((float4 *)(det_rows + (size_t)p * ld))[c] = x;
                ((float4 *)(det_rows + (size_t)(n + p) * ld))[c] = y;
            }
            acc = __builtin_fmaf(x.x, y.x, acc);
            acc = __builtin_fmaf(x.y, y.y, acc);
            acc = __builtin_fmaf(x.z, y.z, acc);
            acc = __builtin_fmaf(x.w, y.w, acc);
        }
        acc += __shfl_xor(acc, 8, 64);
        acc += __shfl_xor(acc, 4, 64);
        acc += __shfl_xor(acc, 2, 64);
        acc += __shfl_xor(acc, 1, 64);
        const float sc = acc + bv;
        const float sg = 1.0f / (1.0f + expf(-sc));
        float ds;
        if (a.is_d) {
            ds = sg - xp;
        } else {
            const bool inside = (sg >= 1e-5f) && (sg <= 1.0f);
            ds = inside ? -(xp * inv_n) * (1.0f - sg) : 0.0f;
        }
        if (t == 0) {
            coef[p] = ds;
            coefb[p] = a.is_d ? ds + a.lambda * bv : ds;
        }
    }
    if (stamp) pw[1] = wall_clock64();
    __syncthreads();
    if (stamp) pw[2] = wall_clock64();
    constexpr int NW = SMALLN ? 2 : 2 * DET_MAX_PAIRS / 64;
    constexpr int NFW = (NF + 3) / 4;
    constexpr int CB = 4;
    const int lane = threadIdx.x & 63;
    const int wave = __builtin_amdgcn_readfirstlane((int)(threadIdx.x >> 6));
    int idr[NW];
#pragma unroll
    for (int j = 0; j < NW; ++j) idr[j] = (64 * j + lane < 2 * n) ? ids[64 * j + lane] : -1;
    auto leader_of = [&](const int s, int &r, uint64_t (&m)[NW]) -> bool {
        r = __builtin_amdgcn_readlane(idr[0], s & 63);
#pragma unroll
        for (int j = 1; j < NW; ++j) r = (s >> 6) == j ? __builtin_amdgcn_readlane(idr[j], s & 63) : r;
        bool earlier = false;
#pragma unroll
        for (int j = 0; j < NW; ++j) {
            m[j] = __ballot(idr[j] == r);
// ... 59 lines not shown
            }
        } else {
            const int64_t ro = (int64_t)r * ld;
#pragma unroll
            for (int i = 0; i < NFW; ++i) {
                const int f = lane + 64 * i;
                if (f < ld) {
                    float var = own[i];
                    if (OPT == 2) {
                        var -= o.lr * acc[i];
                    } else {
                        float m1 = PRE ? pm[i] : o.mE[ro + f], v1 = PRE ? pv[i] : o.vE[ro + f];
                        adam_elem(var, m1, v1, acc[i], o);
                        o.mE[ro + f] = m1;
                        o.vE[ro + f] = v1;
                    }
                    if (!__builtin_isfinite(var)) *o.bad = 1ull;
                    o.E[ro + f] = var;
                }
            }
            if (lane == 0) {
                float var = PRE ? pb[0] : o.b[r];
                if (OPT == 2) {
                    var -= o.lr * accb;
                } else {
                    float m1 = PRE ? pb[1] : o.mb[r], v1 = PRE ? pb[2] : o.vb[r];
                    adam_elem(var, m1, v1, accb, o);
                    o.mb[r] = m1;
                    o.vb[r] = v1;
                }
                if (!__builtin_isfinite(var)) *o.bad = 1ull;
                o.b[r] = var;
            }
        }
    };
    if constexpr (OPT != 0 && SMALLN && NFW <= 2) {
        constexpr int SPW = 2 * 64 / (DET_THREADS / 64);
        constexpr int SPH = SPW / 2;
#pragma clang loop unroll(full)
        for (int h0 = 0; h0 < SPW; h0 += SPH) {
            float pm[SPH][NFW], pv[SPH][NFW], pb[SPH][3];
#pragma clang loop unroll(full)
            for (int k = 0; k < SPH; ++k) {
                const int s = wave + (h0 + k) * (DET_THREADS / 64);
                int r = 0;
                uint64_t m[NW];
#pragma unroll
                for (int i = 0; i < NFW; ++i) { pm[k][i] = 0.f; pv[k][i] = 0.f; }
                pb[k][0] = pb[k][1] = pb[k][2] = 0.f;
                if (s < 2 * n && leader_of(s, r, m)) {
                    const int64_t ro = (int64_t)r * ld;
#pragma unroll
                    for (int i = 0; i < NFW; ++i) {
                        const int f = lane + 64 * i;
                        if (OPT == 1 && f < ld) { pm[k][i] = o.mE[ro + f]; pv[k][i] = o.vE[ro + f]; }
                    }
                    if (lane == 0) {
                        pb[k][0] = o.b[r];
                        if (OPT == 1) { pb[k][1] = o.mb[r]; pb[k][2] = o.vb[r]; }
                    }
                }
            }
#pragma clang loop unroll(full)
            for (int k = 0; k < SPH; ++k) {
                const int s = wave + (h0 + k) * (DET_THREADS / 64);
                int r = 0;
                uint64_t m[NW];
                if (s < 2 * n && leader_of(s, r, m)) own_row(s, r, m, true, pm[k], pv[k], pb[k]);
            }
        }
    } else {
        const float none[NFW] = {}, none3[3] = {};
        for (int s = (int)blockIdx.x * (DET_THREADS / 64) + wave; s < 2 * n; s += (int)gridDim.x * (DET_THREADS / 64)) {
            int r = 0;
            uint64_t m[NW];
            if (leader_of(s, r, m)) own_row(s, r, m, false, none, none, none3);
        }
    }
    if (stamp) pw[3] = wall_clock64();
}

static unsigned det_workgroups(int n) {
    static const int cap = [] { const char *e = getenv("GG_DET_WORKGROUPS"); return e ? std::max(1, atoi(e)) : 8; }();
    return (unsigned)std::min(cap, std::max(1, (2 * n + DET_THREADS / 64 - 1) / (DET_THREADS / 64)));
}

static bool det_lds_granted(int device);
static bool det_rows_fit_lds(const gg_ctx *ctx, const StepArgs &s) {
    return (size_t)2 * s.n * s.ld * sizeof(float) <= DET_LDS_ROW_BYTES && det_lds_granted(ctx->device);
}

template <int NF, int OPT>
static hipError_t launch_pair_grad_det_lds(gg_ctx *ctx, const StepArgs &s, const OptArgs &o) {
    static bool raised_dev[64] = {};
    bool &raised = raised_dev[ctx->device & 63];
    if (!raised) {
        hipError_t e = hipFuncSetAttribute((const void *)pair_grad_det_kernel<NF, true, OPT, true>, hipFuncAttributeMaxDynamicSharedMemorySize, (int)DET_LDS_ROW_BYTES);
        if (e == hipSuccess) e = hipFuncSetAttribute((const void *)pair_grad_det_kernel<NF, true, OPT, false>, hipFuncAttributeMaxDynamicSharedMemorySize, (int)DET_LDS_ROW_BYTES);
        if (e != hipSuccess) return e;
        raised = true;
    }
    const size_t dyn = (size_t)2 * s.n * s.ld * sizeof(float);
    const dim3 grid(OPT == 0 ? det_workgroups(s.n) : 1);
    if (s.n <= 64) hipLaunchKernelGGL((pair_grad_det_kernel<NF, true, OPT, true>), grid, dim3(DET_THREADS), dyn, ctx->stream, s, o);
    else hipLaunchKernelGGL((pair_grad_det_kernel<NF, true, OPT, false>), grid, dim3(DET_THREADS), dyn, ctx->stream, s, o);
    return hipSuccess;
}

static bool det_lds_granted(int device) {
    static int state[64] = {};
    int &s = state[device & 63];
    if (s == 0) {
        const hipError_t e = hipFuncSetAttribute((const void *)pair_grad_det_kernel<4, true, 0, true>, hipFuncAttributeMaxDynamicSharedMemorySize, (int)DET_LDS_ROW_BYTES);
        if (e != hipSuccess) (void)hipGetLastError();
        s = e == hipSuccess ? 1 : -1;
    }
    return s > 0;
}

template <int NF>
static hipError_t launch_pair_grad_det(gg_ctx *ctx, const StepArgs &s, const OptArgs &o, int opt) {
    if (!det_rows_fit_lds(ctx, s)) {
        const dim3 grid(det_workgroups(s.n));
        if (s.n <= 64) hipLaunchKernelGGL((pair_grad_det_kernel<NF, false, 0, true>), grid, dim3(DET_THREADS), 0, ctx->stream, s, o);
        else hipLaunchKernelGGL((pair_grad_det_kernel<NF, false, 0, false>), grid, dim3(DET_THREADS), 0, ctx->stream, s, o);
        return hipSuccess;
    }
    if (opt == 1) return launch_pair_grad_det_lds<NF, 1>(ctx, s, o);
    if (opt == 2) return launch_pair_grad_det_lds<NF, 2>(ctx, s, o);
    return launch_pair_grad_det_lds<NF, 0>(ctx, s, o);
}

template <int SGD>
__global__ __launch_bounds__(256) void sparse_opt_kernel(const OptArgs a) {
    const int t = threadIdx.x & 15;
    const int g0 = (blockIdx.x * blockDim.x + threadIdx.x) >> 4;
    const int ng = (gridDim.x * blockDim.x) >> 4;
    const int cnt = (int)*a.touched_total;
    const int nchunk = a.ld >> 2;
    for (int r = g0; r < cnt; r += ng) opt_row<SGD>(a, a.touched_list[r], t, nchunk);
}

constexpr int STAGE_SORT = 64;

template <int MODE>
__global__ __launch_bounds__(256) void staged_opt_kernel(const OptArgs a) {
    constexpr bool SGD = MODE == 1;
    __shared__ int32_t perm_s[16][STAGE_SORT];
    const int t = threadIdx.x & 15;
    int32_t *const perm = perm_s[threadIdx.x >> 4];
    const int64_t g0 = ((int64_t)blockIdx.x * blockDim.x + threadIdx.x) >> 4, ng = ((int64_t)gridDim.x * blockDim.x) >> 4;
    const int64_t n_rows = a.sg_tot[0];
    const int nchunk = a.ld >> 2;
    for (int64_t r = g0; r < n_rows; r += ng) {
        const int4 e = a.sg_list[r];
        const int row = e.x, n = e.z;
        const float4 *const seg = (const float4 *)(a.stage + (int64_t)e.y * a.ld);
        const float *const sb = a.stage_b + e.y;
        const int32_t *const key = a.stage_key + e.y;
        float4 g[4];
#pragma unroll
        for (int i = 0; i < 4; ++i) g[i] = make_float4(0.f, 0.f, 0.f, 0.f);
        float gbias = 0.f;
        auto add_row = [&](const float4 *src) {
#pragma unroll
            for (int i = 0; i < 4; ++i) {
                const int c = t + 16 * i;
                if (c < nchunk) {
                    const float4 x = src[c];
                    g[i].x += x.x; g[i].y += x.y; g[i].z += x.z; g[i].w += x.w;
                }
            }
        };
        if (n <= STAGE_SORT) {
            if (n > 1) {
                int k[4], rk[4];
#pragma unroll
                for (int i = 0; i < 4; ++i) {
                    k[i] = (t + 16 * i < n) ? key[t + 16 * i] : 0x7fffffff;
                    rk[i] = 0;
                }
#pragma unroll
                for (int j = 0; j < 4; ++j) {
                    if (16 * j < n) {
                        const int nl = min(n - 16 * j, 16);
                        for (int l = 0; l < nl; ++l) {
                            const int kk = __shfl(k[j], l, 16);
#pragma unroll
                            for (int i = 0; i < 4; ++i) rk[i] += kk < k[i];
                        }
                    }
                }
#pragma unroll
                for (int i = 0; i < 4; ++i)
                    if (t + 16 * i < n) perm[rk[i]] = t + 16 * i;
            } else if (t == 0) {
                perm[0] = 0;
            }
            __builtin_amdgcn_fence(__ATOMIC_RELEASE, "wavefront");
            __builtin_amdgcn_wave_barrier();
            __builtin_amdgcn_fence(__ATOMIC_ACQUIRE, "wavefront");
            int o = 0;
            for (; o + 4 <= n; o += 4) {
                const float4 *s0 = seg + (int64_t)perm[o] * nchunk, *s1 = seg + (int64_t)perm[o + 1] * nchunk;
                const float4 *s2 = seg + (int64_t)perm[o + 2] * nchunk, *s3 = seg + (int64_t)perm[o + 3] * nchunk;
#pragma unroll
                for (int i = 0; i < 4; ++i) {
                    const int c = t + 16 * i;
                    if (c < nchunk) {
                        const float4 x0 = s0[c], x1 = s1[c], x2 = s2[c], x3 = s3[c];
                        g[i].x += x0.x; g[i].y += x0.y; g[i].z += x0.z; g[i].w += x0.w;
                        g[i].x += x1.x; g[i].y += x1.y; g[i].z += x1.z; g[i].w += x1.w;
                        g[i].x += x2.x; g[i].y += x2.y; g[i].z += x2.z; g[i].w += x2.w;
                        g[i].x += x3.x; g[i].y += x3.y; g[i].z += x3.z; g[i].w += x3.w;
                    }
                }
            }
            for (; o < n; ++o) add_row(seg + (int64_t)perm[o] * nchunk);
            for (int q = t; q < n; q += 16) gbias += sb[perm[q]];
            __builtin_amdgcn_wave_barrier();
        } else {
            int last = -1;
            for (int q = 0; q < n; ++q) {
                int best = 0x7fffffff, besto = 0;
                for (int o = t; o < n; o += 16) {
                    const int kk = key[o];
                    if (kk > last && kk < best) { best = kk; besto = o; }
                }
#pragma unroll
                for (int m = 8; m >= 1; m >>= 1) {
                    const int ob = __shfl_xor(best, m, 16), oo = __shfl_xor(besto, m, 16);
                    if (ob < best) { best = ob; besto = oo; }
                }
                add_row(seg + (int64_t)besto * nchunk);
                if ((q & 15) == t) gbias += sb[besto];
                last = best;
            }
        }
        gbias += __shfl_xor(gbias, 8, 64);
        gbias += __shfl_xor(gbias, 4, 64);
        gbias += __shfl_xor(gbias, 2, 64);
        gbias += __shfl_xor(gbias, 1, 64);
        const int64_t o4 = ((int64_t)row * a.ld) >> 2;
        if (MODE == 2) {
#pragma unroll
            for (int i = 0; i < 4; ++i) {
                const int c = t + 16 * i;
                if (c < nchunk) ((float4 *)a.gE)[o4 + c] = g[i];
            }
            if (t == 0) {
                a.gb[row] = gbias;
                a.touched[row] = 1;
                a.sg_cnt[row] = 0;
            }
            continue;
        }
#pragma unroll
        for (int i = 0; i < 4; ++i) {
            const int c = t + 16 * i;
            if (c >= nchunk) continue;
            float4 var = ((float4 *)a.E)[o4 + c];
            if (SGD) {
                var.x -= a.lr * g[i].x; var.y -= a.lr * g[i].y; var.z -= a.lr * g[i].z; var.w -= a.lr * g[i].w;
            } else {
                float4 m = ((float4 *)a.mE)[o4 + c], v = ((float4 *)a.vE)[o4 + c];
                adam_elem(var.x, m.x, v.x, g[i].x, a);
                adam_elem(var.y, m.y, v.y, g[i].y, a);
                adam_elem(var.z, m.z, v.z, g[i].z, a);
                adam_elem(var.w, m.w, v.w, g[i].w, a);
                ((float4 *)a.mE)[o4 + c] = m;
                ((float4 *)a.vE)[o4 + c] = v;
            }
            if (nonfinite4(var)) *a.bad = 1ull;
            ((float4 *)a.E)[o4 + c] = var;
        }
        if (t == 0) {
            float var = a.b[row];
            if (SGD) {
                var -= a.lr * gbias;
            } else {
                float m = a.mb[row], v = a.vb[row];
                adam_elem(var, m, v, gbias, a);
                a.mb[row] = m;
                a.vb[row] = v;
            }
            if (!__builtin_isfinite(var)) *a.bad = 1ull;
            a.b[row] = var;
            a.sg_cnt[row] = 0;
        }
    }
}

__global__ void add_word_kernel(int64_t *dst, const int64_t *src) { *dst += *src; }

__global__ __launch_bounds__(256) void pack_rows_kernel(float *gE, float *gb, int32_t *touched, const int32_t *list, const int64_t *cnt_ptr,
                                                        int64_t cap, int ld, int32_t *out_ids, float *out_rows, int32_t *err) {
    const int t = threadIdx.x & 15;
    const int64_t g0 = ((int64_t)blockIdx.x * blockDim.x + threadIdx.x) >> 4, ng = ((int64_t)gridDim.x * blockDim.x) >> 4;
    const int64_t cnt = *cnt_ptr;
    if (cnt > cap && blockIdx.x == 0 && threadIdx.x == 0) *err = 1;
    for (int64_t r = g0; r < cap; r += ng) {
        if (r >= cnt) {
            if (t == 0) out_ids[r] = -1;
            continue;
        }
        const int row = list[r];
        float *src = gE + (int64_t)row * ld, *dst = out_rows + r * (ld + 1);
        for (int f = t; f < ld; f += 16) { dst[f] = src[f]; src[f] = 0.f; }
        if (t == 0) { dst[ld] = gb[row]; gb[row] = 0.f; out_ids[r] = row; touched[row] = 0; }
    }
}

__device__ __forceinline__ uint16_t f32_to_bf16(float x) {
    uint32_t u = __builtin_bit_cast(uint32_t, x);
    if ((u & 0x7fffffffu) > 0x7f800000u) return (uint16_t)((u >> 16) | 0x40u);
    u += 0x7fffu + ((u >> 16) & 1u);
    return (uint16_t)(u >> 16);
}
__device__ __forceinline__ float bf16_to_f32(uint16_t h) { return __builtin_bit_cast(float, (uint32_t)h << 16); }
static inline size_t pack_row_words(int ld, bool bf16) { return bf16 ? (size_t)(ld + 2) / 2 : (size_t)ld + 1; }
template <bool BF16> __device__ __forceinline__ float pack_get(const float *rows, int64_t r, int ld, int f) {
    if (BF16) return bf16_to_f32(((const uint16_t *)rows)[r * (ld + 2) + f]);
    return rows[r * (ld + 1) + f];
}
template <bool BF16> __device__ __forceinline__ void pack_put(float *rows, int64_t r, int ld, int f, float v) {
    if (BF16) ((uint16_t *)rows)[r * (ld + 2) + f] = f32_to_bf16(v);
    else rows[r * (ld + 1) + f] = v;
}

template <bool BF16 = false>
__global__ __launch_bounds__(256) void add_rows_kernel(float *gE, float *gb, int32_t *touched, const int32_t *ids, const float *rows, int64_t cnt,
                                                       int ld) {
    const int t = threadIdx.x & 15;
    const int64_t g0 = ((int64_t)blockIdx.x * blockDim.x + threadIdx.x) >> 4, ng = ((int64_t)gridDim.x * blockDim.x) >> 4;
    for (int64_t r = g0; r < cnt; r += ng) {
        const int row = ids[r];
        if (row < 0) continue;
        float *dst = gE + (int64_t)row * ld;
        for (int f = t; f < ld; f += 16) dst[f] += pack_get<BF16>(rows, r, ld, f);
        if (t == 0) { gb[row] += pack_get<BF16>(rows, r, ld, ld); touched[row] = 1; }
    }
}


int apply_optimizer(gg_ctx *ctx, int which, int64_t n);
void step_done(gg_ctx *ctx, int which, int64_t n);
int run_path_step(gg_ctx *ctx);

static OptArgs make_opt_args(gg_ctx *ctx, int which) {
    Model &M = ctx->model[which];
    OptArgs o{};
    o.E = M.E; o.b = M.b; o.mE = M.mE; o.vE = M.vE; o.mb = M.mb; o.vb = M.vb; o.gE = ctx->gradE; o.gb = ctx->gradb;
    o.nE = (int64_t)ctx->n_node * ctx->ld;
    o.n_node = ctx->n_node; o.ld = ctx->ld;
    o.b1 = ctx->cfg.adam_beta1; o.b2 = ctx->cfg.adam_beta2; o.eps = ctx->cfg.adam_eps;
    o.lr = M.lr;
    o.lr_t = (M.lr * sqrtf(1.0f - M.b2p)) / (1.0f - M.b1p);
    o.touched = ctx->touched; o.touched_list = ctx->touched_list; o.touched_cnt = ctx->touched_cnt;
    o.bad = ctx->table_bad.as<unsigned long long>() + which;
    return o;
}

__global__ void set_count_kernel(int64_t *dst, int64_t v) { *dst = v; }

static int global_pair_count(gg_ctx *ctx, int64_t n_local, const int64_t **out) {
    *out = nullptr;
    const int world = ctx->comm ? ctx->world : ctx->fake_world;
    if (world <= 1) return GG_OK;
    GG_HIP(ctx, ctx->x_nglob.reserve(sizeof(int64_t) * 2));
    int64_t *w = ctx->x_nglob.as<int64_t>();
    hipLaunchKernelGGL(set_count_kernel, dim3(1), dim3(1), 0, ctx->stream, w, ctx->comm ? n_local : n_local * world);
    if (ctx->comm) {
        int rc = comm_allreduce_i64(ctx, w, 1);
        if (rc != GG_OK) return rc;
    }
    *out = w;
    return GG_OK;
}

static int64_t stage_bytes_cap() {
    static const int64_t cap = [] {
        const char *e = getenv("GG_STAGE_MAX_BYTES");
        return e ? (int64_t)atoll(e) : (int64_t)24 << 30;
    }();
    return cap;
}

__global__ __launch_bounds__(256) void hub_index_kernel(const int32_t *cnt, int64_t n, int T, int32_t *off, int32_t *rows, int64_t *nhub) {
    const int64_t i = (int64_t)blockIdx.x * blockDim.x + threadIdx.x;
    if (i >= n || cnt[i] <= T) return;
    const int h = (int)atomicAdd((unsigned long long *)nhub, 1ull);
    off[i] = h;
    rows[h] = (int32_t)i;
}

__global__ __launch_bounds__(256) void hub_finalize_kernel(unsigned long long *acc, const int32_t *rows, const int64_t *nhub, int64_t cap, int ld,
                                                           double inv_scale, float *gE, float *gb) {
    const int64_t n = min(*nhub, cap) * (ld + 1);
    for (int64_t i = (int64_t)blockIdx.x * blockDim.x + threadIdx.x; i < n; i += (int64_t)gridDim.x * blockDim.x) {
        const unsigned long long v = acc[i];
        if (!v) continue;
        acc[i] = 0ull;
        const int64_t h = i / (ld + 1);
        const int f = (int)(i - h * (ld + 1));
        const float x = (float)((double)(long long)v * inv_scale);
        if (f < ld) gE[(int64_t)rows[h] * ld + f] += x;
        else gb[rows[h]] += x;
    }
}

static float hub_scale(bool per_pair_mean, int64_t n) {
    return std::ldexp(1.0f, 32 + (per_pair_mean && n > 1 ? (int)std::ilogb((double)n) : 0));
}

static HubAcc hub_args(gg_ctx *ctx, float scale) {
    return HubAcc{ctx->hub_acc.as<unsigned long long>(), ctx->hub_cap, scale};
}

static int hub_index(gg_ctx *ctx, const int32_t *cnt, int32_t *off, DevBuf &rows, int64_t *tot, hipStream_t stream) {
    GG_HIP(ctx, rows.reserve(sizeof(int32_t) * (size_t)ctx->n_node));
    GG_HIP(ctx, hipMemsetAsync(tot + 2, 0, sizeof(int64_t), stream));
    hipLaunchKernelGGL(hub_index_kernel, dim3((unsigned)cdiv(ctx->n_node, 256)), dim3(256), 0, stream, cnt, (int64_t)ctx->n_node, ctx->sg_threshold, off,
                       rows.as<int32_t>(), tot + 2);
    GG_HIP(ctx, hipGetLastError());
    return GG_OK;
}

static void hub_finalize(gg_ctx *ctx, bool early_index, float scale, float *gE, float *gb) {
    DevBuf &rows = early_index ? ctx->sgp_hub : ctx->sg_hub, &tot = early_index ? ctx->sgp_tot : ctx->sg_tot;
    const int64_t n = ctx->hub_cap * (ctx->ld + 1);
    const unsigned nb = (unsigned)std::max<int64_t>(1, std::min<int64_t>(cdiv(n, 256), 2048));
    hipLaunchKernelGGL(hub_finalize_kernel, dim3(nb), dim3(256), 0, ctx->stream, ctx->hub_acc.as<unsigned long long>(), rows.as<int32_t>(),
                       tot.as<int64_t>() + 2, ctx->hub_cap, ctx->ld, 1.0 / (double)scale, gE, gb);
}

static int staged_reserve(gg_ctx *ctx, int64_t n_occ, int64_t n_stage) {
    if (n_stage * (int64_t)(ctx->ld + 2) * 4 > stage_bytes_cap()) return 1;
    const size_t cnt_before = ctx->sg_cnt.bytes;
    GG_HIP(ctx, ctx->sg_cnt.reserve(sizeof(int32_t) * (size_t)ctx->n_node));
    const bool was_dirty = ctx->sg_cnt_dirty;
    if (ctx->sg_cnt.bytes != cnt_before || ctx->sg_cnt_dirty) GG_HIP(ctx, hipMemsetAsync(ctx->sg_cnt.p, 0, ctx->sg_cnt.bytes, ctx->stream));
    ctx->sg_cnt_dirty = true;
    GG_HIP(ctx, ctx->sg_off.reserve(sizeof(int32_t) * (size_t)ctx->n_node));
    GG_HIP(ctx, ctx->sg_list.reserve(sizeof(int4) * (size_t)ctx->n_node));
    GG_HIP(ctx, ctx->sg_slot.reserve(sizeof(int32_t) * (size_t)n_occ));
    GG_HIP(ctx, ctx->sg_bias.reserve(sizeof(float) * (size_t)n_stage));
    GG_HIP(ctx, ctx->sg_key.reserve(sizeof(int32_t) * (size_t)n_stage));
    GG_HIP(ctx, ctx->sg_tot.reserve(sizeof(int64_t) * 4));
    {
        const int64_t cap = std::min<int64_t>(ctx->n_node, n_occ / ((int64_t)ctx->sg_threshold + 1) + 1);
        const size_t before = ctx->hub_acc.bytes;
        if (ctx->hub_acc.reserve(sizeof(unsigned long long) * (size_t)cap * (ctx->ld + 1)) != hipSuccess) {
            (void)hipGetLastError();
            ctx->hub_cap = 0;
            return 1;
        }
        if (ctx->hub_acc.bytes != before || was_dirty) GG_HIP(ctx, hipMemsetAsync(ctx->hub_acc.p, 0, ctx->hub_acc.bytes, ctx->stream));
        ctx->hub_cap = (int64_t)(ctx->hub_acc.bytes / (sizeof(unsigned long long) * (ctx->ld + 1)));
    }
    if (ctx->sg_rows.reserve(sizeof(float) * (size_t)n_stage * ctx->ld) != hipSuccess) {
        (void)hipGetLastError();
        return 1;
    }
    return GG_OK;
}

static int staged_finish(gg_ctx *ctx, int which, int64_t n, int64_t n_occ, bool early_index = false) {
    const int opt = ctx->cfg.optimizer;
    OptArgs o = make_opt_args(ctx, which);
    DevBuf &b_cnt = early_index ? ctx->sgp_cnt : ctx->sg_cnt, &b_list = early_index ? ctx->sgp_list : ctx->sg_list;
    DevBuf &b_tot = early_index ? ctx->sgp_tot : ctx->sg_tot, &b_key = early_index ? ctx->sgp_key : ctx->sg_key;
    o.sg_cnt = b_cnt.as<int32_t>(); o.sg_list = b_list.as<int4>(); o.sg_tot = b_tot.as<int64_t>();
    o.stage = ctx->sg_rows.as<float>(); o.stage_b = ctx->sg_bias.as<float>(); o.stage_key = b_key.as<int32_t>();
    int nb = cdiv((int64_t)std::min<int64_t>(n_occ, ctx->n_node) * 16, 256);
    if (nb > 4096) nb = 4096;
    if (nb < 1) nb = 1;
    const bool replicas = ctx->comm || ctx->fake_world > 1;
    if (replicas) hipLaunchKernelGGL(staged_opt_kernel<2>, dim3(nb), dim3(256), 0, ctx->stream, o);
    else if (opt == GG_OPT_SGD) hipLaunchKernelGGL(staged_opt_kernel<1>, dim3(nb), dim3(256), 0, ctx->stream, o);
    else hipLaunchKernelGGL(staged_opt_kernel<0>, dim3(nb), dim3(256), 0, ctx->stream, o);
    ctx->sg_active = true;
    ctx->sg_cnt_active = o.sg_cnt;
    const int rc = apply_optimizer(ctx, which, n);
    ctx->sg_active = false;
    if (rc != GG_OK) return rc;
    if (!replicas)
        hipLaunchKernelGGL(add_word_kernel, dim3(1), dim3(1), 0, ctx->stream, ctx->touched_ptr.as<int64_t>() + ctx->n_node, b_tot.as<int64_t>());
    GG_HIP(ctx, hipGetLastError());
    if (early_index) ctx->sgp_cnt_clean = true;
    else ctx->sg_cnt_dirty = false;
    return GG_OK;
}

static bool staged_allowed(const gg_ctx *ctx) {
    return ctx->sg_threshold > 0 && ctx->ld <= 256 && ctx->cfg.optimizer != GG_OPT_ADAM_DENSE && !getenv("GG_NO_STAGED_GRAD");
}

int run_step(gg_ctx *ctx, int which, const int32_t *d_u, const int32_t *d_v, const float *d_x, int32_t n) {
    if (n <= 0) return GG_OK;
    Model &M = ctx->model[which];
    const int opt = ctx->cfg.optimizer;
    StepArgs s{};
    s.E = M.E; s.b = M.b; s.gE = ctx->gradE; s.gb = ctx->gradb;
    s.touched = ctx->touched; s.touched_list = ctx->touched_list; s.touched_cnt = ctx->touched_cnt;
    s.ld = ctx->ld;
    s.track = opt != GG_OPT_ADAM_DENSE;
    s.u = d_u; s.v = d_v; s.x = d_x; s.n = n;
    s.lambda = M.lambda;
    s.inv_n = 1.0f / (float)n;
    s.is_d = which == 1;
    if (which == 0) {
        int rc = global_pair_count(ctx, n, &s.n_glob);
        if (rc != GG_OK) return rc;
    }
    s.ppg = n >= 16384 ? PAIRS_PER_GROUP : (n >= 2048 ? 4 : 1);
    if (ctx->deterministic && n <= DET_MAX_PAIRS) {
        const int nfd = (ctx->ld + 15) / 16;
        const bool replicas = ctx->comm || ctx->fake_world > 1;
        const int fused = (!replicas && opt != GG_OPT_ADAM_DENSE && det_rows_fit_lds(ctx, s) && !getenv("GG_NO_FUSED_SMALL_STEP")) ? (opt == GG_OPT_SGD ? 2 : 1) : 0;
        const OptArgs o = make_opt_args(ctx, which);
        static unsigned long long *det_prof = nullptr;
        static const bool det_prof_on = getenv("GG_DET_PROFILE") != nullptr;
        if (det_prof_on) {
            if (!det_prof) GG_HIP(ctx, hipMalloc((void **)&det_prof, 16 * sizeof(unsigned long long)));
            GG_HIP(ctx, hipMemsetAsync(det_prof, 0, 16 * sizeof(unsigned long long), ctx->stream));
            s.prof = det_prof;
        }
        hipError_t e;
        if (nfd <= 4) e = launch_pair_grad_det<4>(ctx, s, o, fused);
        else if (nfd <= 8) e = launch_pair_grad_det<8>(ctx, s, o, fused);
        else if (nfd <= 16) e = launch_pair_grad_det<16>(ctx, s, o, fused);
        else e = launch_pair_grad_det<32>(ctx, s, o, fused);
        GG_HIP(ctx, e);
        if (det_prof_on) {
            static double acc_t[2][2][4] = {};
            static long cnt[2] = {};
            unsigned long long h[16];
            GG_HIP(ctx, hipMemcpyAsync(h, det_prof, sizeof(h), hipMemcpyDeviceToHost, ctx->stream));
            GG_HIP(ctx, hipStreamSynchronize(ctx->stream));
            for (int w = 0; w < 2; ++w)
                for (int k = 0; k < 3; ++k) acc_t[which][w][k] += h[8 * w + k + 1] > h[8 * w + k] ? 10.0 * (double)(h[8 * w + k + 1] - h[8 * w + k]) : 0.0;
            if (++cnt[which] % 1000 == 0)
                for (int w = 0; w < 2; ++w)
                    fprintf(stderr, "[det] model %d n=%d wave %s: loads+coef %.0f ns, barrier %.0f, owners' sums + stores issued %.0f (means over %ld steps)\n", which, n, w ? "15" : "0",
                            acc_t[which][w][0] / cnt[which], acc_t[which][w][1] / cnt[which], acc_t[which][w][2] / cnt[which], cnt[which]);
        }
        if (fused) {
            GG_HIP(ctx, hipGetLastError());
            step_done(ctx, which, n);
            return GG_OK;
        }
        return apply_optimizer(ctx, which, n);
    }
    const int groups = cdiv(n, s.ppg);
    const int blocks = cdiv((int64_t)groups * 16, 256);
    const int nf = (ctx->ld + 15) / 16;
    bool staged = n >= 16384 && n < (1 << 30) && staged_allowed(ctx);
    if (staged) {
        int rc = staged_reserve(ctx, 2 * (int64_t)n, 2 * (int64_t)n);
        if (rc < 0) return rc;
        if (rc == 1) staged = false;
    }
    if (staged) {
        int rc;
        int32_t *cnt = ctx->sg_cnt.as<int32_t>(), *off = ctx->sg_off.as<int32_t>(), *slot_v = ctx->sg_slot.as<int32_t>(), *slot_u = slot_v + n;
        hipLaunchKernelGGL(pair_occ_count_kernel, dim3(cdiv(n, 256)), dim3(256), 0, ctx->stream, d_u, d_v, n, s.ppg, cnt, slot_v, slot_u);
        rc = device_segment_rows(ctx, cnt, ctx->n_node, ctx->sg_threshold, off, ctx->sg_list.as<int4>(), ctx->sg_tot.as<int64_t>());
        if (rc != GG_OK) return rc;
        rc = hub_index(ctx, cnt, off, ctx->sg_hub, ctx->sg_tot.as<int64_t>(), ctx->stream);
        if (rc != GG_OK) return rc;
        hipLaunchKernelGGL(pair_occ_slot_kernel, dim3(cdiv(n, 256)), dim3(256), 0, ctx->stream, d_u, d_v, n, cnt, off, ctx->sg_threshold, slot_v, slot_u,
                           ctx->sg_key.as<int32_t>());
        s.slot_v = slot_v; s.slot_u = slot_u;
        s.stage = ctx->sg_rows.as<float>(); s.stage_b = ctx->sg_bias.as<float>();
        const float scale = hub_scale(!s.is_d, n);
        s.hub = hub_args(ctx, scale);
        if (nf <= 4) hipLaunchKernelGGL((pair_grad16_kernel<4, true>), dim3(blocks), dim3(256), 0, ctx->stream, s);
        else if (nf <= 8) hipLaunchKernelGGL((pair_grad16_kernel<8, true>), dim3(blocks), dim3(256), 0, ctx->stream, s);
        else hipLaunchKernelGGL((pair_grad16_kernel<16, true>), dim3(blocks), dim3(256), 0, ctx->stream, s);
        hub_finalize(ctx, false, scale, s.gE, s.gb);
        if (ctx->tm_cur >= 0) GG_HIP(ctx, hipEventRecord(ctx->tm_ev[ctx->tm_cur][1], ctx->stream));
        return staged_finish(ctx, which, n, 2 * (int64_t)n);
    }
    if (s.ppg == PAIRS_PER_GROUP && nf <= 16 && !getenv("GG_OLD_PAIR_GRAD")) {
        if (nf <= 4) hipLaunchKernelGGL((pair_grad16_kernel<4, false>), dim3(blocks), dim3(256), 0, ctx->stream, s);
        else if (nf <= 8) hipLaunchKernelGGL((pair_grad16_kernel<8, false>), dim3(blocks), dim3(256), 0, ctx->stream, s);
        else hipLaunchKernelGGL((pair_grad16_kernel<16, false>), dim3(blocks), dim3(256), 0, ctx->stream, s);
    } else if (nf <= 4) hipLaunchKernelGGL((pair_grad_kernel<4, false>), dim3(blocks), dim3(256), 0, ctx->stream, s);
    else if (nf <= 8) hipLaunchKernelGGL((pair_grad_kernel<8, false>), dim3(blocks), dim3(256), 0, ctx->stream, s);
    else if (nf <= 16) hipLaunchKernelGGL((pair_grad_kernel<16, false>), dim3(blocks), dim3(256), 0, ctx->stream, s);
    else hipLaunchKernelGGL((pair_grad_kernel<32, false>), dim3(blocks), dim3(256), 0, ctx->stream, s);
    if (ctx->tm_cur >= 0) GG_HIP(ctx, hipEventRecord(ctx->tm_ev[ctx->tm_cur][1], ctx->stream));

    return apply_optimizer(ctx, which, n);
}

template <bool STAGED>
static void launch_path_grad(gg_ctx *ctx, const PathArgs &p, int blocks, int nf) {
    const dim3 g(blocks), b(256);
    if (p.stride <= 17) {
        if (nf <= 4) hipLaunchKernelGGL((path_grad_kernel<4, STAGED, true>), g, b, 0, ctx->stream, p);
        else if (nf <= 8) hipLaunchKernelGGL((path_grad_kernel<8, STAGED, true>), g, b, 0, ctx->stream, p);
        else hipLaunchKernelGGL((path_grad_kernel<16, STAGED, true>), g, b, 0, ctx->stream, p);
    } else {
        if (nf <= 4) hipLaunchKernelGGL((path_grad_kernel<4, STAGED, false>), g, b, 0, ctx->stream, p);
        else if (nf <= 8) hipLaunchKernelGGL((path_grad_kernel<8, STAGED, false>), g, b, 0, ctx->stream, p);
        else hipLaunchKernelGGL((path_grad_kernel<16, STAGED, false>), g, b, 0, ctx->stream, p);
    }
}

int run_path_step(gg_ctx *ctx) {
    Model &M = ctx->model[0];
    const int64_t n = ctx->g_pairs;
    PathArgs p{};
    p.E = M.E; p.b = M.b; p.gE = ctx->gradE; p.gb = ctx->gradb;
    p.touched = ctx->touched; p.touched_list = ctx->touched_list; p.touched_cnt = ctx->touched_cnt;
    p.ld = ctx->ld;
    p.track = ctx->cfg.optimizer != GG_OPT_ADAM_DENSE;
    p.window = ctx->cfg.window_size;
    p.paths = ctx->w_paths.as<int32_t>();
    p.path_len = ctx->w_len.as<int32_t>();
    p.stride = ctx->w_stride;
    p.pair_ptr = ctx->g_ptr.as<int64_t>();
    p.reward = ctx->g_reward.as<float>();
    p.n_walks = ctx->w_total;
    p.lambda = M.lambda;
    p.inv_n = 1.0f / (float)n;
    {
        int rc = global_pair_count(ctx, n, &p.n_glob);
        if (rc != GG_OK) return rc;
    }
    const int blocks = cdiv(p.n_walks * 16, 256);
    const int nf = (ctx->ld + 15) / 16;
    const int64_t n_pos = p.n_walks * (int64_t)p.stride;
    bool staged = staged_allowed(ctx) && n_pos < (1ll << 31);
    const int64_t n_stage = std::min<int64_t>(n_pos, p.window >= 2 ? (n + 6 * p.n_walks) / 4 + 1 : (n + 2 * p.n_walks) / 2 + 1);
    if (staged) {
        const int rc = staged_reserve(ctx, n_pos, n_stage);
        if (rc < 0) return rc;
        if (rc == 1) staged = false;
    }
    if (!staged) {
        launch_path_grad<false>(ctx, p, blocks, nf);
        if (ctx->tm_cur >= 0) GG_HIP(ctx, hipEventRecord(ctx->tm_ev[ctx->tm_cur][1], ctx->stream));
        return apply_optimizer(ctx, 0, n);
    }
    int rc;
    int32_t *cnt = ctx->sg_cnt.as<int32_t>(), *off = ctx->sg_off.as<int32_t>(), *slot = ctx->sg_slot.as<int32_t>();
    const dim3 pgrid((unsigned)cdiv(n_pos, 256));
    const bool early = ctx->g_slots_ready && ctx->g_slots_walks == p.n_walks && ctx->g_slots_stride == p.stride;
    ctx->g_slots_ready = false;
    ctx->g_slots_unused = 0;
    if (early) {
        ctx->sg_cnt_dirty = false;
        GG_HIP(ctx, hipStreamWaitEvent(ctx->stream, ctx->ev_slots_done, 0));
        slot = ctx->sgp_slot.as<int32_t>();
    } else {
        hipLaunchKernelGGL(path_count_kernel, pgrid, dim3(256), 0, ctx->stream, p.paths, p.path_len, p.stride, p.n_walks, cnt, slot, (const unsigned long long *)nullptr);
        rc = device_segment_rows(ctx, cnt, ctx->n_node, ctx->sg_threshold, off, ctx->sg_list.as<int4>(), ctx->sg_tot.as<int64_t>());
        if (rc != GG_OK) return rc;
        rc = hub_index(ctx, cnt, off, ctx->sg_hub, ctx->sg_tot.as<int64_t>(), ctx->stream);
        if (rc != GG_OK) return rc;
        hipLaunchKernelGGL(path_slot_kernel, pgrid, dim3(256), 0, ctx->stream, p.paths, p.path_len, p.stride, p.n_walks, cnt, off, ctx->sg_threshold, slot,
                           ctx->sg_key.as<int32_t>(), (const unsigned long long *)nullptr);
    }
    p.slot = slot;
    p.stage = ctx->sg_rows.as<float>();
    p.stage_b = ctx->sg_bias.as<float>();
    const float scale = hub_scale(true, n);
    p.hub = hub_args(ctx, scale);
    launch_path_grad<true>(ctx, p, blocks, nf);
    hub_finalize(ctx, early, scale, p.gE, p.gb);
    if (ctx->tm_cur >= 0) GG_HIP(ctx, hipEventRecord(ctx->tm_ev[ctx->tm_cur][1], ctx->stream));
    return staged_finish(ctx, 0, n, n_pos, early);
}

int enqueue_path_slots(gg_ctx *ctx) {
    ctx->g_slots_ready = false;
    if (ctx->walk_stream == ctx->stream || ctx->in_epoch_add || getenv("GG_NO_EARLY_SLOTS")) return GG_OK;
    const int64_t n_walks = ctx->w_total, n_pos = n_walks * (int64_t)ctx->w_stride;
    if (!staged_allowed(ctx) || ctx->cfg.window_size > 2 || n_walks == 0 || n_pos >= (1ll << 31)) return GG_OK;
    if (ctx->g_slots_unused >= 2) {
        if (ctx->sgp_slot.p) {
            for (DevBuf *b : {&ctx->sgp_cnt, &ctx->sgp_off, &ctx->sgp_slot, &ctx->sgp_list, &ctx->sgp_key, &ctx->sgp_scan, &ctx->sgp_hub}) b->release();
            ctx->sgp_cnt_clean = false;
        }
        return GG_OK;
    }
    hipStream_t st = ctx->walk_stream;
    const size_t cnt_before = ctx->sgp_cnt.bytes;
    GG_HIP(ctx, ctx->sgp_cnt.reserve(sizeof(int32_t) * (size_t)ctx->n_node));
    if (ctx->sgp_cnt.bytes != cnt_before || !ctx->sgp_cnt_clean) GG_HIP(ctx, hipMemsetAsync(ctx->sgp_cnt.p, 0, ctx->sgp_cnt.bytes, st));
    ctx->sgp_cnt_clean = false;
    GG_HIP(ctx, ctx->sgp_off.reserve(sizeof(int32_t) * (size_t)ctx->n_node));
    GG_HIP(ctx, ctx->sgp_list.reserve(sizeof(int4) * (size_t)ctx->n_node));
    GG_HIP(ctx, ctx->sgp_slot.reserve(sizeof(int32_t) * (size_t)n_pos));
    GG_HIP(ctx, ctx->sgp_key.reserve(sizeof(int32_t) * (size_t)n_pos));
    GG_HIP(ctx, ctx->sgp_tot.reserve(sizeof(int64_t) * 4));
    if (!ctx->ev_slots_done) GG_HIP(ctx, hipEventCreateWithFlags(&ctx->ev_slots_done, hipEventDisableTiming));
    const unsigned long long *flag = ctx->dev_ctr + 3;
    const dim3 pgrid((unsigned)cdiv(n_pos, 256));
    int32_t *cnt = ctx->sgp_cnt.as<int32_t>(), *off = ctx->sgp_off.as<int32_t>(), *slot = ctx->sgp_slot.as<int32_t>();
    hipLaunchKernelGGL(path_count_kernel, pgrid, dim3(256), 0, st, ctx->w_paths.as<int32_t>(), ctx->w_len.as<int32_t>(), ctx->w_stride, n_walks, cnt, slot, flag);
    int rc = device_segment_rows(ctx, cnt, ctx->n_node, ctx->sg_threshold, off, ctx->sgp_list.as<int4>(), ctx->sgp_tot.as<int64_t>(), st, &ctx->sgp_scan);
    if (rc != GG_OK) return rc;
    rc = hub_index(ctx, cnt, off, ctx->sgp_hub, ctx->sgp_tot.as<int64_t>(), st);
    if (rc != GG_OK) return rc;
    hipLaunchKernelGGL(path_slot_kernel, pgrid, dim3(256), 0, st, ctx->w_paths.as<int32_t>(), ctx->w_len.as<int32_t>(), ctx->w_stride, n_walks, cnt, off,
                       ctx->sg_threshold, slot, ctx->sgp_key.as<int32_t>(), flag);
    GG_HIP(ctx, hipGetLastError());
    GG_HIP(ctx, hipEventRecord(ctx->ev_slots_done, st));
    ctx->g_slots_ready = true;
    ctx->g_slots_walks = n_walks;
    ctx->g_slots_stride = ctx->w_stride;
    return GG_OK;
}

__global__ void normalize_flags_kernel(int32_t *f, int n) {
    const int i = blockIdx.x * blockDim.x + threadIdx.x;
    if (i < n && f[i] > 1) f[i] = 1;
}

__global__ void scale_grads_kernel(float *gE, float *gb, int64_t nE, int n, float k) {
    const int64_t stride = (int64_t)gridDim.x * blockDim.x;
    for (int64_t i = (int64_t)blockIdx.x * blockDim.x + threadIdx.x; i < nE; i += stride) gE[i] *= k;
    for (int64_t i = (int64_t)blockIdx.x * blockDim.x + threadIdx.x; i < n; i += stride) gb[i] *= k;
}

__global__ __launch_bounds__(256) void owner_count_kernel(const int32_t *list, const int64_t *cnt_ptr, int world, long long *cnt) {
    __shared__ int sh[64];
    if (threadIdx.x < 64) sh[threadIdx.x] = 0;
    __syncthreads();
    const int64_t n = *cnt_ptr;
    for (int64_t i = (int64_t)blockIdx.x * blockDim.x + threadIdx.x; i < n; i += (int64_t)gridDim.x * blockDim.x) atomicAdd(&sh[list[i] % world], 1);
    __syncthreads();
    if ((int)threadIdx.x < world && sh[threadIdx.x]) atomicAdd((unsigned long long *)&cnt[threadIdx.x], (unsigned long long)sh[threadIdx.x]);
}

template <bool BF16>
__global__ __launch_bounds__(256) void owner_pack_kernel(const float *gE, const float *gb, const int32_t *list, const int64_t *cnt_ptr, int world,
                                                         const long long *seg_off, long long *fill, int ld, int32_t *out_ids, float *out_rows) {
    const int t = threadIdx.x & 15;
    const int64_t g0 = ((int64_t)blockIdx.x * blockDim.x + threadIdx.x) >> 4, ng = ((int64_t)gridDim.x * blockDim.x) >> 4;
    const int64_t cnt = *cnt_ptr;
    for (int64_t r = g0; r < cnt; r += ng) {
        const int row = list[r];
        const int q = row % world;
        long long slot = 0;
        if (t == 0) slot = seg_off[q] + (long long)atomicAdd((unsigned long long *)&fill[q], 1ull);
        slot = __shfl(slot, (threadIdx.x & 63) & ~15, 64);
        const float *src = gE + (int64_t)row * ld;
        for (int f = t; f < ld; f += 16) pack_put<BF16>(out_rows, slot, ld, f, src[f]);
        if (t == 0) {
            pack_put<BF16>(out_rows, slot, ld, ld, gb[row]);
            if (BF16) pack_put<BF16>(out_rows, slot, ld, ld + 1, 0.f);
            out_ids[slot] = row;
        }
    }
}

template <bool BF16>
__global__ __launch_bounds__(256) void owner_gather_pack_kernel(float *gE, float *gb, const int32_t *list, const int64_t *cnt_ptr, int world,
                                                                int me, long long *fill, int64_t cap, int ld, int32_t *out_ids, float *out_rows) {
    const int t = threadIdx.x & 15;
    const int64_t g0 = ((int64_t)blockIdx.x * blockDim.x + threadIdx.x) >> 4, ng = ((int64_t)gridDim.x * blockDim.x) >> 4;
    const int64_t cnt = *cnt_ptr;
    for (int64_t r = g0; r < cnt; r += ng) {
        const int row = list[r];
        if (row % world != me) continue;
        long long slot = 0;
        if (t == 0) slot = (long long)atomicAdd((unsigned long long *)fill, 1ull);
        slot = __shfl(slot, (threadIdx.x & 63) & ~15, 64);
        if (slot >= cap) continue;
        float *src = gE + (int64_t)row * ld;
        for (int f = t; f < ld; f += 16) {
            pack_put<BF16>(out_rows, slot, ld, f, src[f]);
            if (BF16) src[f] = pack_get<BF16>(out_rows, slot, ld, f);
        }
        if (t == 0) {
            pack_put<BF16>(out_rows, slot, ld, ld, gb[row]);
            if (BF16) { gb[row] = pack_get<BF16>(out_rows, slot, ld, ld); pack_put<BF16>(out_rows, slot, ld, ld + 1, 0.f); }
            out_ids[slot] = row;
        }
    }
}

__global__ void owner_count_owned_kernel(const int32_t *list, const int64_t *cnt_ptr, int world, int me, long long *out) {
    const int64_t n = *cnt_ptr;
    int c = 0;
    for (int64_t i = (int64_t)blockIdx.x * blockDim.x + threadIdx.x; i < n; i += (int64_t)gridDim.x * blockDim.x) c += (list[i] % world == me) ? 1 : 0;
    for (int off = 32; off >= 1; off >>= 1) c += __shfl_xor(c, off, 64);
    if ((threadIdx.x & 63) == 0 && c) atomicAdd((unsigned long long *)out, (unsigned long long)c);
}

__global__ void fill_ids_kernel(int32_t *ids, int64_t n, int32_t v) {
    for (int64_t i = (int64_t)blockIdx.x * blockDim.x + threadIdx.x; i < n; i += (int64_t)gridDim.x * blockDim.x) ids[i] = v;
}

template <bool BF16>
__global__ __launch_bounds__(256) void set_rows_kernel(float *gE, float *gb, int32_t *touched, const int32_t *ids, const float *rows, int64_t cnt, int ld) {
    const int t = threadIdx.x & 15;
    const int64_t g0 = ((int64_t)blockIdx.x * blockDim.x + threadIdx.x) >> 4, ng = ((int64_t)gridDim.x * blockDim.x) >> 4;
    for (int64_t r = g0; r < cnt; r += ng) {
        const int row = ids[r];
        if (row < 0) continue;
        float *dst = gE + (int64_t)row * ld;
        for (int f = t; f < ld; f += 16) dst[f] = pack_get<BF16>(rows, r, ld, f);
        if (t == 0) { gb[row] = pack_get<BF16>(rows, r, ld, ld); touched[row] = 1; }
    }
}

static int exchange_owner(gg_ctx *ctx, OptArgs &o, int world, bool *taken) {
    *taken = false;
    const int n = ctx->n_node, ld = ctx->ld;
    const bool fake = !ctx->comm;
    if (!ctx->owner_exchange || world < 2 || world > 64 || !comm_has_p2p(ctx)) return GG_OK;
    const bool bf16 = ctx->comm_bf16;
    const size_t row_f = pack_row_words(ld, bf16);
    int rc = device_compact_flags(ctx, ctx->touched, n, ctx->touched_list, ctx->touched_ptr.as<int64_t>() + n);
    if (rc != GG_OK) return rc;
    GG_HIP(ctx, ctx->x_own.reserve(sizeof(long long) * (size_t)(3 * world + world * world + 8)));
    long long *cnt = ctx->x_own.as<long long>(), *fill = cnt + world, *seg = cnt + 2 * world, *mat = cnt + 3 * world, *own = mat + world * world;
    GG_HIP(ctx, hipMemsetAsync(cnt, 0, sizeof(long long) * (size_t)(3 * world + world * world + 8), ctx->stream));
    hipLaunchKernelGGL(owner_count_kernel, dim3(256), dim3(256), 0, ctx->stream, ctx->touched_list, o.touched_total, world, cnt);
    rc = comm_allgather(ctx, cnt, mat, (size_t)world, 8);
    if (rc != GG_OK) return rc;
    std::vector<long long> M((size_t)world * world);
    GG_HIP(ctx, hipMemcpyAsync(M.data(), mat, sizeof(long long) * M.size(), hipMemcpyDeviceToHost, ctx->stream));
    GG_HIP(ctx, hipStreamSynchronize(ctx->stream));
    const int me_real = fake ? 0 : ctx->rank;
    long long sum_t = 0, max_t = 0;
    for (int r = 0; r < world; ++r) {
        long long tr = 0;
        for (int q = 0; q < world; ++q) tr += M[(size_t)r * world + q];
        sum_t += tr;
        max_t = std::max(max_t, tr);
    }
    const double f = (double)(world - 1) / world;
    if (f * (double)max_t + f * (double)std::min<long long>(n, sum_t) >= 0.9 * 2.0 * f * (double)n) return GG_OK;
    std::vector<long long> soff(world + 1, 0);
    for (int q = 0; q < world; ++q) soff[q + 1] = soff[q] + M[(size_t)me_real * world + q];
    const long long T = soff[world];
    GG_HIP(ctx, hipMemcpyAsync(seg, soff.data(), sizeof(long long) * world, hipMemcpyHostToDevice, ctx->stream));
    GG_HIP(ctx, ctx->x_send_ids.reserve(sizeof(int32_t) * (size_t)std::max<long long>(T, 1)));
    GG_HIP(ctx, ctx->x_send_rows.reserve(sizeof(float) * (size_t)std::max<long long>(T, 1) * row_f));
    int nb = cdiv(std::max<long long>(T, 1) * 16, 256);
    if (nb > 4096) nb = 4096;
    if (bf16) hipLaunchKernelGGL(owner_pack_kernel<true>, dim3(nb), dim3(256), 0, ctx->stream, ctx->gradE, ctx->gradb, ctx->touched_list, o.touched_total, world, seg, fill, ld,
                                 ctx->x_send_ids.as<int32_t>(), ctx->x_send_rows.as<float>());
    else hipLaunchKernelGGL(owner_pack_kernel<false>, dim3(nb), dim3(256), 0, ctx->stream, ctx->gradE, ctx->gradb, ctx->touched_list, o.touched_total, world, seg, fill, ld,
                            ctx->x_send_ids.as<int32_t>(), ctx->x_send_rows.as<float>());
    long long bytes = 0;
    const int owners = fake ? world : 1;
    for (int oi = 0; oi < owners; ++oi) {
        const int me = fake ? oi : ctx->rank;
        std::vector<int64_t> s_off(world, 0), s_cnt(world, 0), r_off(world, 0), r_cnt(world, 0), si_off(world, 0), si_cnt(world, 0), ri_off(world, 0), ri_cnt(world, 0);
        long long R = 0;
        for (int r = 0; r < world; ++r) {
            if (r == me) continue;
            const long long in = M[(size_t)r * world + me], out = M[(size_t)me * world + r];
            ri_off[r] = R; ri_cnt[r] = in;
            r_off[r] = R * (long long)row_f; r_cnt[r] = in * (long long)row_f;
// ... 334 lines not shown
```

### graphgan_amd/engine.py

```python
from __future__ import annotations

import ctypes

import numpy as np

from . import _lib
from ._lib import GGConfig, GGCounters, check, lib


def _ptr(a):
    return None if a is None else a.ctypes.data_as(ctypes.c_void_p)


def _i32(a):
    return np.ascontiguousarray(a, dtype=np.int32)


def graph_to_csr(n_node, graph):
    deg = np.fromiter((len(graph.get(v, ())) for v in range(n_node)), dtype=np.int64, count=n_node)
    rowptr = np.zeros(n_node + 1, dtype=np.int64)
    np.cumsum(deg, out=rowptr[1:])
    col = np.empty(int(rowptr[-1]), dtype=np.int32)
    for v in range(n_node):
        lst = graph.get(v)
# ... 403 lines not shown
        ms = ctypes.c_double()
        self._ck(lib.gg_topk_scores(self._ctx, which, _ptr(rows_a), n_rows, k, {"fp32": 0, "bf16": 1}[precision], int(bool(exclude)),
                                    _ptr(col), _ptr(score), ctypes.byref(ms)))
        return dict(col=col, score=score, kernel_ms=ms.value)

    def graph_softmax(self, slots, for_d=False, nodes=None, q3_store=False):
        slots_a = np.asarray(slots)
        if slots_a.ndim != 1 or (slots_a.size and not np.issubdtype(slots_a.dtype, np.integer)):
            raise ValueError("graph_softmax: slots must be a 1-d array of integers")
        slots_a = _i32(slots_a)
        R = len(self.tree_roots)
        if slots_a.size and (int(slots_a.min()) < 0 or int(slots_a.max()) >= R):
            raise ValueError("graph_softmax: slot outside [0, %d)" % R)
        ns = len(slots_a)
        flags = (_lib.GG_GS_FOR_D if for_d else 0) | (_lib.GG_GS_Q3_STORE if q3_store else 0)
        abort = np.zeros(ns, dtype=np.float32)
        ms = ctypes.c_double()
        if nodes is None:
            logp = np.empty((ns, self.n_node), dtype=np.float32)
            self._ck(lib.gg_graph_softmax(self._ctx, _ptr(slots_a), ns, flags, _ptr(logp), None, None, None, _ptr(abort), ctypes.byref(ms)))
            self.last_graph_softmax_ms = ms.value
            return logp, abort
        per_slot = isinstance(nodes, list)
        if per_slot:
            if len(nodes) != ns:
                raise ValueError("graph_softmax: %d node lists for %d slots" % (len(nodes), ns))
            lists = [np.asarray(x).reshape(-1) for x in nodes]
            off = np.zeros(ns + 1, dtype=np.int64)
            np.cumsum([len(x) for x in lists], out=off[1:])
            flat = np.concatenate(lists) if lists else np.zeros(0, np.int64)
        else:
            if not (isinstance(nodes, tuple) and len(nodes) == 2):
                raise ValueError("graph_softmax: nodes must be a list of per-slot arrays or a tuple (flat node ids, offsets)")
            flat, off = np.asarray(nodes[0]).reshape(-1), np.asarray(nodes[1]).reshape(-1)
            if len(off) != ns + 1 or (len(off) and (off[0] != 0 or off[-1] != len(flat) or np.any(np.diff(off) < 0))):
                raise ValueError("graph_softmax: offsets must be [n_slots + 1], monotone, from 0 to len(nodes)")
            off = np.ascontiguousarray(off, dtype=np.int64)
        if flat.size and (not np.issubdtype(flat.dtype, np.integer) or int(flat.min()) < 0 or int(flat.max()) >= self.n_node):
            raise ValueError("graph_softmax: node id outside [0, %d)" % self.n_node)
        flat = _i32(flat)
        q = np.empty(len(flat), dtype=np.float32)
        self._ck(lib.gg_graph_softmax(self._ctx, _ptr(slots_a), ns, flags, None, _ptr(off), _ptr(flat), _ptr(q), _ptr(abort), ctypes.byref(ms)))
        self.last_graph_softmax_ms = ms.value
        if per_slot:
            return [q[off[k]:off[k + 1]] for k in range(ns)], abort
        return q, abort

    def _nc_args(self, fn, nodes, which, n_class, labels=None):
        if which not in (0, 1):
            raise ValueError("%s: which must be 0 (generator) or 1 (discriminator), got %r" % (fn, which))
        if isinstance(n_class, bool) or int(n_class) != n_class or not 2 <= int(n_class) <= 128:
            raise ValueError("%s: n_class must be an integer in [2, 128], got %r" % (fn, n_class))
        nodes_a = np.asarray(nodes)
        if nodes_a.ndim != 1 or nodes_a.size == 0 or not np.issubdtype(nodes_a.dtype, np.integer):
            raise ValueError("%s: nodes must be a non-empty 1-d array of integers" % fn)
        if int(nodes_a.min()) < 0 or int(nodes_a.max()) >= self.n_node:
            raise ValueError("%s: node id outside [0, %d)" % (fn, self.n_node))
        if labels is None:
            return _i32(nodes_a), None
        labels_a = np.asarray(labels)
        if labels_a.shape != nodes_a.shape or not np.issubdtype(labels_a.dtype, np.integer):
            raise ValueError("%s: labels must be integers, one per node" % fn)
        if int(labels_a.min()) < 0 or int(labels_a.max()) >= int(n_class):
            raise ValueError("%s: label outside [0, n_class = %d)" % (fn, int(n_class)))
        return _i32(nodes_a), _i32(labels_a)

    def _nc_params(self, fn, W, b):
        W = np.ascontiguousarray(W, dtype=np.float32)
        b = np.ascontiguousarray(b, dtype=np.float32)
        if W.ndim != 2 or W.shape[1] != self.n_emb or b.shape != (W.shape[0],):
            raise ValueError("%s: W must be [n_class, %d] and b [n_class], got %r and %r" % (fn, self.n_emb, W.shape, b.shape))
        return W, b

    def classifier_lossgrad(self, nodes, labels, W, b, which=0, l2=0.0):
        W, b = self._nc_params("classifier_lossgrad", W, b)
        C = int(W.shape[0])
        nodes_a, labels_a = self._nc_args("classifier_lossgrad", nodes, which, C, labels)
        loss = np.zeros(1, dtype=np.float32)
        gW = np.empty_like(W)
        gb = np.empty_like(b)
        self._ck(lib.gg_classifier_lossgrad(self._ctx, which, _ptr(nodes_a), _ptr(labels_a), len(nodes_a), C, _ptr(W), _ptr(b), float(l2),
                                            _ptr(loss), _ptr(gW), _ptr(gb)))
        return dict(loss=float(loss[0]), gW=gW, gb=gb)

    def classifier_fit(self, nodes, labels, n_class, which=0, iters=200, lr=0.05, l2=1e-4, W=None, b=None):
        nodes_a, labels_a = self._nc_args("classifier_fit", nodes, which, n_class, labels)
        C = int(n_class)
        if isinstance(iters, bool) or int(iters) != iters or int(iters) < 1:
            raise ValueError("classifier_fit: iters must be an integer >= 1, got %r" % (iters,))
        if not (np.isfinite(lr) and lr > 0) or not (np.isfinite(l2) and l2 >= 0):
            raise ValueError("classifier_fit: lr must be > 0 and l2 >= 0, got %r and %r" % (lr, l2))
        if (W is None) != (b is None):
            raise ValueError("classifier_fit: give both W and b, or neither")
        if W is None:
            W, b = np.zeros((C, self.n_emb), dtype=np.float32), np.zeros(C, dtype=np.float32)
        else:
            W, b = self._nc_params("classifier_fit", W, b)
            if W.shape[0] != C:
                raise ValueError("classifier_fit: W has %d rows, n_class is %d" % (W.shape[0], C))
            W, b = W.copy(), b.copy()
        loss = np.empty(int(iters), dtype=np.float32)
        ms = ctypes.c_double()
        self._ck(lib.gg_classifier_fit(self._ctx, which, _ptr(nodes_a), _ptr(labels_a), len(nodes_a), C, int(iters), float(lr), float(l2),
                                       _ptr(W), _ptr(b), _ptr(loss), ctypes.byref(ms)))
        return dict(W=W, b=b, loss=loss, ms=ms.value)

    def classifier_predict(self, nodes, W, b, which=0, logits=False):
        W, b = self._nc_params("classifier_predict", W, b)
        C = int(W.shape[0])
        nodes_a, _ = self._nc_args("classifier_predict", nodes, which, C)
        pred = np.empty(len(nodes_a), dtype=np.int32)
        z = np.empty((len(nodes_a), C), dtype=np.float32) if logits else None
        self._ck(lib.gg_classifier_predict(self._ctx, which, _ptr(nodes_a), len(nodes_a), C, _ptr(W), _ptr(b), _ptr(pred), _ptr(z)))
        return (pred, z) if logits else pred

    def get_embeddings(self, which):
        out = np.zeros((self.n_node, self.n_emb), dtype=np.float32)
        self._ck(lib.gg_get_embeddings(self._ctx, which, _ptr(out)))
        return out

    def write_embeddings(self, which, path, n_threads=0):
        self._ck(lib.gg_write_embeddings(self._ctx, which, str(path).encode(), n_threads))

    def write_embeddings_bin(self, which, path):
        self._ck(lib.gg_write_embeddings_bin(self._ctx, which, str(path).encode()))

    def edge_scores(self, which, u, v):
        u, v = _i32(u), _i32(v)
        out = np.zeros(len(u), dtype=np.float64)
        self._ck(lib.gg_edge_scores(self._ctx, which, _ptr(u), _ptr(v), len(u), _ptr(out)))
        return out

    def get_bias(self, which):
        out = np.zeros(self.n_node, dtype=np.float32)
        self._ck(lib.gg_get_bias(self._ctx, which, _ptr(out)))
        return out

    def set_embeddings(self, which, emb):
        emb = np.ascontiguousarray(emb, dtype=np.float32)
        assert emb.shape == (self.n_node, self.n_emb)
        self._ck(lib.gg_set_embeddings(self._ctx, which, _ptr(emb)))

    def set_bias(self, which, bias):
        bias = np.ascontiguousarray(bias, dtype=np.float32)
        assert bias.shape == (self.n_node,)
        self._ck(lib.gg_set_bias(self._ctx, which, _ptr(bias)))

    def save_state(self, path):
        self._ck(lib.gg_save_state(self._ctx, path.encode()))

    def load_state(self, path):
        self._ck(lib.gg_load_state(self._ctx, path.encode()))

    def counters(self):
        c = GGCounters()
        self._ck(lib.gg_get_counters(self._ctx, ctypes.byref(c)))
        return {k: getattr(c, k) for k, _ in GGCounters._fields_ if k != "reserved"}

    def set_profiling(self, every_n):
        self._ck(lib.gg_set_profiling(self._ctx, int(every_n)))

    def set_profiling_solo(self, solo):
        self._ck(lib.gg_set_profiling_solo(self._ctx, int(bool(solo))))

    def synchronize(self):
        self._ck(lib.gg_synchronize(self._ctx))

    @staticmethod
    def comm_unique_id():
        buf = (ctypes.c_char * 128)()
        check(lib.gg_comm_unique_id(buf))
        return bytes(buf)

    def comm_init(self, unique_id, rank, world):
        buf = (ctypes.c_char * 128).from_buffer_copy(unique_id)
        self._ck(lib.gg_comm_init(self._ctx, buf, rank, world))

    def comm_stats(self):
        out = np.zeros(8, dtype=np.int64)
        self._ck(lib.gg_comm_stats_ex(self._ctx, _ptr(out)))
        return dict(sparse_steps=int(out[0] + out[1]), dense_steps=int(out[2]), bytes_sent=int(out[3]), world=int(out[4]),
                    pack_steps=int(out[0]), owner_steps=int(out[1]), bf16_rows=bool(out[5]))

    def comm_barrier(self):
        self._ck(lib.gg_comm_barrier(self._ctx))
```

Baseline: 633.7 million.

## Apply optimizer inline for rows touched exactly once, bypassing staging

Rows whose occurrence count is one are no longer staged. The step kernels apply the Adam or SGD update to them directly, writing E/bias, the moments and the cleared count in place, which removes their staging writes and their later pass through the staged optimizer. The staged optimizer kernel also prefetches the next segment entry and the E/m/v rows before reducing gradients. Per-pass stage statistics counters are added. The fast path is on by default (with an env switch to disable) and off for replicated or comm setups. It adds branching and register pressure to the hot step kernels.

```diff
diff --git a/graphgan_amd/csrc/gg_api.hip b/graphgan_amd/csrc/gg_api.hip
--- a/graphgan_amd/csrc/gg_api.hip
+++ b/graphgan_amd/csrc/gg_api.hip
@@ -375,6 +375,7 @@
     if (const char *nc = getenv("GG_NO_DIST_CACHE")) ctx->dc_enabled = atoi(nc) == 0;
     if (const char *ft = getenv("GG_FIN_THRESHOLD")) ctx->fin_threshold = std::max(0, atoi(ft));
     if (const char *st = getenv("GG_STAGE_T")) ctx->sg_threshold = std::max(0, atoi(st));
+    if (const char *ns = getenv("GG_NO_SINGLE_ROWS")) ctx->single_rows = atoi(ns) == 0;
     if (const char *ws = getenv("GG_WALK_SPLIT")) ctx->split_enabled = atoi(ws) != 0;
     if (const char *em = getenv("GG_ES_MODE")) ctx->es_mode = std::min(2, std::max(0, atoi(em)));
     if (const char *er = getenv("GG_ES_RATIO")) ctx->es_ratio_num = std::max(1, atoi(er));
diff --git a/graphgan_amd/csrc/gg_internal.h b/graphgan_amd/csrc/gg_internal.h
--- a/graphgan_amd/csrc/gg_internal.h
+++ b/graphgan_amd/csrc/gg_internal.h
@@ -193,6 +193,7 @@
     int32_t g_slots_stride = 0;
     int32_t *sg_cnt_active = nullptr;
     bool sg_active = false;
+    bool single_rows = true;
     int sg_threshold = 64;
 
     unsigned long long *dev_ctr = nullptr;
@@ -255,7 +256,7 @@
 int device_exclusive_scan(gg_ctx *ctx, const int32_t *cnt, int64_t *ptr, int64_t n);
 int ensure_g_pairs(gg_ctx *ctx);
 int device_compact_flags(gg_ctx *ctx, const int32_t *flag, int64_t n, int32_t *list, int64_t *total_out);
-int device_segment_rows(gg_ctx *ctx, const int32_t *cnt, int64_t n, int T, int32_t *off, int4 *list, int64_t *totals, hipStream_t stream = nullptr,
+int device_segment_rows(gg_ctx *ctx, const int32_t *cnt, int64_t n, int lo, int T, int32_t *off, int4 *list, int64_t *totals, hipStream_t stream = nullptr,
                         DevBuf *scratch = nullptr);
 
 int alloc_trees(gg_ctx *ctx, const int32_t *roots, int32_t n_roots, const int64_t *node_counts, const int64_t *root_children, int64_t extra_nodes = 0);
diff --git a/graphgan_amd/csrc/prepare.hip b/graphgan_amd/csrc/prepare.hip
--- a/graphgan_amd/csrc/prepare.hip
+++ b/graphgan_amd/csrc/prepare.hip
@@ -149,24 +149,27 @@
     return GG_OK;
 }
 
-__global__ __launch_bounds__(SCAN_THREADS) void seg_tile_sums(const int32_t *cnt, int64_t n, int T, int64_t *tile_rows, int64_t *tile_occ) {
+__global__ __launch_bounds__(SCAN_THREADS) void seg_tile_sums(const int32_t *cnt, int64_t n, int lo, int T, int64_t *tile_rows, int64_t *tile_occ, int64_t *singles) {
     __shared__ int64_t sh[SCAN_THREADS / 64];
     const int64_t base = (int64_t)blockIdx.x * SCAN_TILE + (int64_t)threadIdx.x * SCAN_ITEMS;
-    int64_t rows = 0, occ = 0;
+    int64_t rows = 0, occ = 0, one = 0;
 #pragma unroll
     for (int i = 0; i < SCAN_ITEMS; ++i)
         if (base + i < n) {
             const int c = cnt[base + i];
-            if (c > 0 && c <= T) { rows += 1; occ += c; }
+            if (c >= lo && c <= T) { rows += 1; occ += c; }
+            if (c == 1 && lo > 1) one += 1;
         }
     int64_t tot;
+    (void)block_excl_scan(one, &tot, sh);
+    if (threadIdx.x == 0 && tot) atomicAdd((unsigned long long *)singles, (unsigned long long)tot);
     (void)block_excl_scan(rows, &tot, sh);
     if (threadIdx.x == 0) tile_rows[blockIdx.x] = tot;
     (void)block_excl_scan(occ, &tot, sh);
     if (threadIdx.x == 0) tile_occ[blockIdx.x] = tot;
 }
 
-__global__ __launch_bounds__(SCAN_THREADS) void seg_apply(const int32_t *cnt, int64_t n, int T, const int64_t *tile_rows, const int64_t *tile_occ,
+__global__ __launch_bounds__(SCAN_THREADS) void seg_apply(const int32_t *cnt, int64_t n, int lo, int T, const int64_t *tile_rows, const int64_t *tile_occ,
                                                           int32_t *off, int4 *list) {
     __shared__ int64_t sh[SCAN_THREADS / 64];
     const int64_t base = (int64_t)blockIdx.x * SCAN_TILE + (int64_t)threadIdx.x * SCAN_ITEMS;
@@ -175,7 +178,7 @@
 #pragma unroll
     for (int i = 0; i < SCAN_ITEMS; ++i) {
         const int v = base + i < n ? cnt[base + i] : 0;
-        c[i] = (v > 0 && v <= T) ? v : 0;
+        c[i] = (v >= lo && v <= T) ? v : 0;
         rows += c[i] ? 1 : 0;
         occ += c[i];
     }
@@ -191,15 +194,16 @@
         }
 }
 
-int device_segment_rows(gg_ctx *ctx, const int32_t *cnt, int64_t n, int T, int32_t *off, int4 *list, int64_t *totals, hipStream_t stream, DevBuf *scratch) {
+int device_segment_rows(gg_ctx *ctx, const int32_t *cnt, int64_t n, int lo, int T, int32_t *off, int4 *list, int64_t *totals, hipStream_t stream, DevBuf *scratch) {
     const int64_t tiles = (n + SCAN_TILE - 1) / SCAN_TILE;
     if (!scratch) scratch = &ctx->scan_tmp;
     if (!stream) stream = ctx->stream;
     GG_HIP(ctx, scratch->reserve(sizeof(int64_t) * (2 * tiles + 4)));
     int64_t *tr = scratch->as<int64_t>(), *to = tr + tiles + 1;
-    hipLaunchKernelGGL(seg_tile_sums, dim3((unsigned)tiles), dim3(SCAN_THREADS), 0, stream, cnt, n, T, tr, to);
+    GG_HIP(ctx, hipMemsetAsync(totals + 3, 0, sizeof(int64_t), stream));
+    hipLaunchKernelGGL(seg_tile_sums, dim3((unsigned)tiles), dim3(SCAN_THREADS), 0, stream, cnt, n, lo, T, tr, to, totals + 3);
     hipLaunchKernelGGL(scan_tile_offsets2, dim3(2), dim3(SCAN_THREADS), 0, stream, tr, to, tiles, totals, totals + 1);
-    hipLaunchKernelGGL(seg_apply, dim3((unsigned)tiles), dim3(SCAN_THREADS), 0, stream, cnt, n, T, tr, to, off, list);
+    hipLaunchKernelGGL(seg_apply, dim3((unsigned)tiles), dim3(SCAN_THREADS), 0, stream, cnt, n, lo, T, tr, to, off, list);
     GG_HIP(ctx, hipGetLastError());
     return GG_OK;
 }
diff --git a/graphgan_amd/csrc/steps.hip b/graphgan_amd/csrc/steps.hip
--- a/graphgan_amd/csrc/steps.hip
+++ b/graphgan_amd/csrc/steps.hip
@@ -19,6 +19,63 @@
 }
 __device__ __forceinline__ void hub_add(unsigned long long *p, float x, float scale) {
     atomicAdd(p, (unsigned long long)__float2ll_rn(x * scale));
+}
+
+struct RowOpt {
+    float *mE, *vE, *mb, *vb;
+    int32_t *sg_cnt;
+    unsigned long long *bad;
+    float lr_t, b1, b2, eps, lr;
+    int mode;
+};
+
+template <class A>
+__device__ __forceinline__ void adam_elem(float &var, float &m, float &v, float g, const A &a) {
+    m = m * a.b1;
+    m = m + (1.0f - a.b1) * g;
+    v = v * a.b2;
+    v = v + (g * g) * (1.0f - a.b2);
+    var = var - (a.lr_t * m) / (sqrtf(v) + a.eps);
+}
+
+template <int NF>
+__device__ __forceinline__ void single_apply(const RowOpt &o, float *E, float *b, int row, int ld, int t, const float (&e)[NF], const float (&g)[NF],
+                                             float gbias, float ebias) {
+    float *pe = E + (int64_t)row * ld, *pm = o.mE + (int64_t)row * ld, *pv = o.vE + (int64_t)row * ld;
+    bool bad = false;
+#pragma unroll
+    for (int i = 0; i < NF; ++i) {
+        const int f = t + 16 * i;
+        if (f >= ld) continue;
+        const float gi = 0.f + g[i];
+        float var = e[i];
+        if (o.mode == 2) {
+            var -= o.lr * gi;
+        } else {
+            float m = pm[f], v = pv[f];
+            adam_elem(var, m, v, gi, o);
+            pm[f] = m;
+            pv[f] = v;
+        }
+        bad |= !__builtin_isfinite(var);
+        pe[f] = var;
+    }
+    if (t == 0) {
+        const float gb = 0.f + gbias;
+        float var = ebias;
+        if (o.mode == 2) {
+            var -= o.lr * gb;
+        } else {
+            float m = o.mb[row], v = o.vb[row];
+            adam_elem(var, m, v, gb, o);
+            o.mb[row] = m;
+            o.vb[row] = v;
+        }
+        bad |= !__builtin_isfinite(var);
+        b[row] = var;
+        o.sg_cnt[row] = 0;
+    }
+    if (bad) *o.bad = 1ull;
 }
 
 struct StepArgs {
@@ -37,6 +94,7 @@
     const int32_t *slot_v, *slot_u;
     float *stage, *stage_b;
     HubAcc hub;
+    RowOpt so;
 };
 
 __global__ __launch_bounds__(256) void pair_occ_count_kernel(const int32_t *u, const int32_t *v, int n, int ppg, int32_t *cnt,
@@ -49,15 +107,16 @@
 }
 
 __global__ __launch_bounds__(256) void pair_occ_slot_kernel(const int32_t *u, const int32_t *v, int n, const int32_t *cnt, const int32_t *off,
-                                                            int T, int32_t *slot_v, int32_t *slot_u, int32_t *key) {
+                                                            int T, bool single, int32_t *slot_v, int32_t *slot_u, int32_t *key) {
     const int p = blockIdx.x * blockDim.x + threadIdx.x;
     if (p >= n) return;
     const int iv = v[p], iu = u[p];
-    const int sv = cnt[iv] <= T ? off[iv] + slot_v[p] : -3 - off[iv];
+    const int cv = cnt[iv], cu = cnt[iu];
+    const int sv = (single && cv == 1) ? -2 : (cv <= T ? off[iv] + slot_v[p] : -3 - off[iv]);
     slot_v[p] = sv;
     if (sv >= 0) key[sv] = 2 * p + 1;
     if (slot_u[p] != -2) {
-        const int su = cnt[iu] <= T ? off[iu] + slot_u[p] : -3 - off[iu];
+        const int su = (single && cu == 1) ? -2 : (cu <= T ? off[iu] + slot_u[p] : -3 - off[iu]);
         slot_u[p] = su;
         if (su >= 0) key[su] = 2 * p;
     }
@@ -196,6 +255,12 @@
         for (int r = 0; r < 3; ++r) {
             const int j = j0 + r;
             if (j >= np) break;
+            const int iv = __shfl(myv, j, 16), iu = __shfl(myu, j, 16);
+            const int slv = __shfl(my_sv, j, 16), slu = __shfl(my_su, j, 16);
+            const bool run_ends = __shfl((int)my_end, j, 16) != 0;
+            const bool one_v = STAGED && a.so.mode && slv == -2, one_u = STAGED && a.so.mode && run_ends && slu == -2;
+            float bu = 0.f;
+            if (one_u) bu = a.b[iu];
             fetch(j + 2, U[(r + 2) % 3], V[(r + 2) % 3]);
             float acc = 0.f;
 #pragma unroll
@@ -219,34 +284,44 @@
                 const bool inside = (sg >= 1e-5f) && (sg <= 1.0f);
                 ds = inside ? -(xj * inv_n) * (1.0f - sg) : 0.0f;
             }
-            const int iv = __shfl(myv, j, 16), iu = __shfl(myu, j, 16);
-            const int slv = __shfl(my_sv, j, 16), slu = __shfl(my_su, j, 16);
             const bool st = STAGED && slv >= 0;
             unsigned long long *hv = STAGED && !st ? hub_row(a.hub, slv, a.ld) : nullptr;
             float *gv = st ? a.stage + (int64_t)slv * a.ld : a.gE + (int64_t)iv * a.ld;
-#pragma unroll
-            for (int i = 0; i < NF; ++i) {
-                const int f = t + 16 * i;
-                if (f < a.ld) {
+            const float gbv = a.is_d ? ds + a.lambda * bv : ds;
+            if (one_v) {
+                float gval[NF];
+#pragma unroll
+                for (int i = 0; i < NF; ++i) {
                     accu[i] += ds * V[r][i] + a.lambda * U[r][i];
-                    const float gval = ds * U[r][i] + a.lambda * V[r][i];
-                    if (st) gv[f] = gval;
-                    else if (STAGED && hv) hub_add(hv + f, gval, a.hub.scale);
-                    else atomicAdd(gv + f, gval);
+                    gval[i] = ds * U[r][i] + a.lambda * V[r][i];
                 }
-            }
-            if (t == 0) {
-                const float gbv = a.is_d ? ds + a.lambda * bv : ds;
-                if (st) {
-                    a.stage_b[slv] = gbv;
-                } else {
-                    if (STAGED && hv) hub_add(hv + a.ld, gbv, a.hub.scale);
-                    else atomicAdd(a.gb + iv, gbv);
-                    if (a.track) a.touched[iv] = 1;
+                single_apply<NF>(a.so, a.E, a.b, iv, a.ld, t, V[r], gval, gbv, bv);
+            } else {
+#pragma unroll
+                for (int i = 0; i < NF; ++i) {
+                    const int f = t + 16 * i;
+                    if (f < a.ld) {
+                        accu[i] += ds * V[r][i] + a.lambda * U[r][i];
+                        const float gval = ds * U[r][i] + a.lambda * V[r][i];
+                        if (st) gv[f] = gval;
+                        else if (STAGED && hv) hub_add(hv + f, gval, a.hub.scale);
+                        else atomicAdd(gv + f, gval);
+                    }
                 }
-            }
-            if (__shfl((int)my_end, j, 16)) {
-                if (STAGED && slu >= 0) {
+                if (t == 0) {
+                    if (st) {
+                        a.stage_b[slv] = gbv;
+                    } else {
+                        if (STAGED && hv) hub_add(hv + a.ld, gbv, a.hub.scale);
+                        else atomicAdd(a.gb + iv, gbv);
+                        if (a.track) a.touched[iv] = 1;
+                    }
+                }
+            }
+            if (run_ends) {
+                if (one_u) {
+                    single_apply<NF>(a.so, a.E, a.b, iu, a.ld, t, U[r], accu, 0.f, bu);
+                } else if (STAGED && slu >= 0) {
                     float *gu = a.stage + (int64_t)slu * a.ld;
 #pragma unroll
                     for (int i = 0; i < NF; ++i) {
@@ -288,6 +363,7 @@
     const int32_t *slot;
     float *stage, *stage_b;
     HubAcc hub;
+    RowOpt so;
 };
 
 __global__ __launch_bounds__(256) void path_count_kernel(const int32_t *paths, const int32_t *path_len, int stride, int64_t n_walks,
@@ -301,14 +377,16 @@
 }
 
 __global__ __launch_bounds__(256) void path_slot_kernel(const int32_t *paths, const int32_t *path_len, int stride, int64_t n_walks,
-                                                        const int32_t *cnt, const int32_t *off, int T, int32_t *slot, int32_t *key, const unsigned long long *flag) {
+                                                        const int32_t *cnt, const int32_t *off, int T, bool single, int32_t *slot, int32_t *key,
+                                                        const unsigned long long *flag) {
     const int64_t idx = (int64_t)blockIdx.x * blockDim.x + threadIdx.x;
     const int64_t w = idx / stride;
     if (w >= n_walks || (flag && *flag == 2ull)) return;
     const int c = (int)(idx - w * stride), L = path_len[w] - 1;
     if (L <= 1 || c >= L) return;
     const int nd = paths[idx];
-    const int sl = cnt[nd] <= T ? off[nd] + slot[idx] : -3 - off[nd];
+    const int cn = cnt[nd];
+    const int sl = (single && cn == 1) ? -2 : (cn <= T ? off[nd] + slot[idx] : -3 - off[nd]);
     slot[idx] = sl;
     if (sl >= 0) key[sl] = (int32_t)idx;
 }
@@ -389,6 +467,10 @@
         const float lam_n = a.lambda * npair[sl];
 #pragma unroll
         for (int i = 0; i < NF; ++i) A[sl][i] = __builtin_fmaf(lam_n, R[sl][i], A[sl][i]);
+        if (STAGED && a.so.mode && sslot[sl] == -2) {
+            single_apply<NF>(a.so, a.E, a.b, nd, a.ld, t, R[sl], A[sl], gb[sl], bv[sl]);
+            return;
+        }
         if (STAGED && sslot[sl] >= 0) {
             float *g = a.stage + (int64_t)sslot[sl] * a.ld;
 #pragma unroll
@@ -511,13 +593,6 @@
 
 __device__ __forceinline__ bool nonfinite4(const float4 &x) { return !(__builtin_isfinite(x.x) && __builtin_isfinite(x.y) && __builtin_isfinite(x.z) && __builtin_isfinite(x.w)); }
 
-__device__ __forceinline__ void adam_elem(float &var, float &m, float &v, float g, const OptArgs &a) {
-    m = m * a.b1;
-    m = m + (1.0f - a.b1) * g;
-    v = v * a.b2;
-    v = v + (g * g) * (1.0f - a.b2);
-    var = var - (a.lr_t * m) / (sqrtf(v) + a.eps);
-}
 
 __global__ __launch_bounds__(256) void adam_dense_kernel(const OptArgs a) {
     const int64_t n4 = a.nE >> 2;
@@ -883,12 +958,32 @@
     const int64_t g0 = ((int64_t)blockIdx.x * blockDim.x + threadIdx.x) >> 4, ng = ((int64_t)gridDim.x * blockDim.x) >> 4;
     const int64_t n_rows = a.sg_tot[0];
     const int nchunk = a.ld >> 2;
-    for (int64_t r = g0; r < n_rows; r += ng) {
-        const int4 e = a.sg_list[r];
+    int4 e = g0 < n_rows ? a.sg_list[g0] : make_int4(0, 0, 0, 0), e_next = e;
+    for (int64_t r = g0; r < n_rows; r += ng, e = e_next) {
+        if (r + ng < n_rows) e_next = a.sg_list[r + ng];
         const int row = e.x, n = e.z;
         const float4 *const seg = (const float4 *)(a.stage + (int64_t)e.y * a.ld);
         const float *const sb = a.stage_b + e.y;
         const int32_t *const key = a.stage_key + e.y;
+        const int64_t o4 = ((int64_t)row * a.ld) >> 2;
+        int k[4];
+#pragma unroll
+        for (int i = 0; i < 4; ++i) k[i] = (n > 1 && n <= STAGE_SORT && t + 16 * i < n) ? key[t + 16 * i] : 0x7fffffff;
+        const float4 z4 = make_float4(0.f, 0.f, 0.f, 0.f);
+        float4 pe[4], pm[4], pv[4];
+        float pb = 0.f, pmb = 0.f, pvb = 0.f;
+#pragma unroll
+        for (int i = 0; i < 4; ++i) {
+            const int c = t + 16 * i;
+            const bool in = MODE != 2 && c < nchunk;
+            pe[i] = in ? ((const float4 *)a.E)[o4 + c] : z4;
+            pm[i] = (in && !SGD) ? ((const float4 *)a.mE)[o4 + c] : z4;
+            pv[i] = (in && !SGD) ? ((const float4 *)a.vE)[o4 + c] : z4;
+        }
+        if (MODE != 2 && t == 0) {
+            pb = a.b[row];
+            if (!SGD) { pmb = a.mb[row]; pvb = a.vb[row]; }
+        }
         float4 g[4];
 #pragma unroll
         for (int i = 0; i < 4; ++i) g[i] = make_float4(0.f, 0.f, 0.f, 0.f);
@@ -905,12 +1000,9 @@
         };
         if (n <= STAGE_SORT) {
             if (n > 1) {
-                int k[4], rk[4];
-#pragma unroll
-                for (int i = 0; i < 4; ++i) {
-                    k[i] = (t + 16 * i < n) ? key[t + 16 * i] : 0x7fffffff;
-                    rk[i] = 0;
-                }
+                int rk[4];
+#pragma unroll
+                for (int i = 0; i < 4; ++i) rk[i] = 0;
 #pragma unroll
                 for (int j = 0; j < 4; ++j) {
                     if (16 * j < n) {
@@ -972,7 +1064,6 @@
         gbias += __shfl_xor(gbias, 4, 64);
         gbias += __shfl_xor(gbias, 2, 64);
         gbias += __shfl_xor(gbias, 1, 64);
-        const int64_t o4 = ((int64_t)row * a.ld) >> 2;
         if (MODE == 2) {
 #pragma unroll
             for (int i = 0; i < 4; ++i) {
@@ -990,11 +1081,11 @@
         for (int i = 0; i < 4; ++i) {
             const int c = t + 16 * i;
             if (c >= nchunk) continue;
-            float4 var = ((float4 *)a.E)[o4 + c];
+            float4 var = pe[i];
             if (SGD) {
                 var.x -= a.lr * g[i].x; var.y -= a.lr * g[i].y; var.z -= a.lr * g[i].z; var.w -= a.lr * g[i].w;
             } else {
-                float4 m = ((float4 *)a.mE)[o4 + c], v = ((float4 *)a.vE)[o4 + c];
+                float4 m = pm[i], v = pv[i];
                 adam_elem(var.x, m.x, v.x, g[i].x, a);
                 adam_elem(var.y, m.y, v.y, g[i].y, a);
                 adam_elem(var.z, m.z, v.z, g[i].z, a);
@@ -1006,11 +1097,11 @@
             ((float4 *)a.E)[o4 + c] = var;
         }
         if (t == 0) {
-            float var = a.b[row];
+            float var = pb;
             if (SGD) {
                 var -= a.lr * gbias;
             } else {
-                float m = a.mb[row], v = a.vb[row];
+                float m = pmb, v = pvb;
                 adam_elem(var, m, v, gbias, a);
                 a.mb[row] = m;
                 a.vb[row] = v;
@@ -1022,7 +1113,11 @@
     }
 }
 
-__global__ void add_word_kernel(int64_t *dst, const int64_t *src) { *dst += *src; }
+__global__ void pass_totals_kernel(int64_t *dst, const int64_t *tot, unsigned long long *stat) {
+    if (dst) *dst += tot[0] + tot[3];
+    for (int k = 0; k < 4; ++k) stat[k] += (unsigned long long)tot[k];
+    stat[4] += 1ull;
+}
 
 __global__ __launch_bounds__(256) void pack_rows_kernel(float *gE, float *gb, int32_t *touched, const int32_t *list, const int64_t *cnt_ptr,
                                                         int64_t cap, int ld, int32_t *out_ids, float *out_rows, int32_t *err) {
@@ -1196,6 +1291,20 @@
     return GG_OK;
 }
 
+static bool staged_replicas(const gg_ctx *ctx) { return ctx->comm || ctx->fake_world > 1; }
+static bool single_rows_on(const gg_ctx *ctx) { return ctx->single_rows && !staged_replicas(ctx); }
+
+static RowOpt single_row_args(gg_ctx *ctx, int which, int32_t *cnt) {
+    const OptArgs o = make_opt_args(ctx, which);
+    RowOpt r{};
+    r.mE = o.mE; r.vE = o.vE; r.mb = o.mb; r.vb = o.vb;
+    r.sg_cnt = cnt;
+    r.bad = o.bad;
+    r.lr_t = o.lr_t; r.b1 = o.b1; r.b2 = o.b2; r.eps = o.eps; r.lr = o.lr;
+    r.mode = !single_rows_on(ctx) ? 0 : (ctx->cfg.optimizer == GG_OPT_SGD ? 2 : 1);
+    return r;
+}
+
 static int staged_finish(gg_ctx *ctx, int which, int64_t n, int64_t n_occ, bool early_index = false) {
     const int opt = ctx->cfg.optimizer;
     OptArgs o = make_opt_args(ctx, which);
@@ -1206,7 +1315,7 @@
     int nb = cdiv((int64_t)std::min<int64_t>(n_occ, ctx->n_node) * 16, 256);
     if (nb > 4096) nb = 4096;
     if (nb < 1) nb = 1;
-    const bool replicas = ctx->comm || ctx->fake_world > 1;
+    const bool replicas = staged_replicas(ctx);
     if (replicas) hipLaunchKernelGGL(staged_opt_kernel<2>, dim3(nb), dim3(256), 0, ctx->stream, o);
     else if (opt == GG_OPT_SGD) hipLaunchKernelGGL(staged_opt_kernel<1>, dim3(nb), dim3(256), 0, ctx->stream, o);
     else hipLaunchKernelGGL(staged_opt_kernel<0>, dim3(nb), dim3(256), 0, ctx->stream, o);
@@ -1215,8 +1324,8 @@
     const int rc = apply_optimizer(ctx, which, n);
     ctx->sg_active = false;
     if (rc != GG_OK) return rc;
-    if (!replicas)
-        hipLaunchKernelGGL(add_word_kernel, dim3(1), dim3(1), 0, ctx->stream, ctx->touched_ptr.as<int64_t>() + ctx->n_node, b_tot.as<int64_t>());
+    hipLaunchKernelGGL(pass_totals_kernel, dim3(1), dim3(1), 0, ctx->stream, replicas ? nullptr : ctx->touched_ptr.as<int64_t>() + ctx->n_node,
+                       b_tot.as<int64_t>(), ctx->dev_ctr + 1600 + 8 * which);
     GG_HIP(ctx, hipGetLastError());
     if (early_index) ctx->sgp_cnt_clean = true;
     else ctx->sg_cnt_dirty = false;
@@ -1296,12 +1405,14 @@
         int rc;
         int32_t *cnt = ctx->sg_cnt.as<int32_t>(), *off = ctx->sg_off.as<int32_t>(), *slot_v = ctx->sg_slot.as<int32_t>(), *slot_u = slot_v + n;
         hipLaunchKernelGGL(pair_occ_count_kernel, dim3(cdiv(n, 256)), dim3(256), 0, ctx->stream, d_u, d_v, n, s.ppg, cnt, slot_v, slot_u);
-        rc = device_segment_rows(ctx, cnt, ctx->n_node, ctx->sg_threshold, off, ctx->sg_list.as<int4>(), ctx->sg_tot.as<int64_t>());
+        const bool single = single_rows_on(ctx);
+        rc = device_segment_rows(ctx, cnt, ctx->n_node, single ? 2 : 1, ctx->sg_threshold, off, ctx->sg_list.as<int4>(), ctx->sg_tot.as<int64_t>());
         if (rc != GG_OK) return rc;
         rc = hub_index(ctx, cnt, off, ctx->sg_hub, ctx->sg_tot.as<int64_t>(), ctx->stream);
         if (rc != GG_OK) return rc;
-        hipLaunchKernelGGL(pair_occ_slot_kernel, dim3(cdiv(n, 256)), dim3(256), 0, ctx->stream, d_u, d_v, n, cnt, off, ctx->sg_threshold, slot_v, slot_u,
-                           ctx->sg_key.as<int32_t>());
+        hipLaunchKernelGGL(pair_occ_slot_kernel, dim3(cdiv(n, 256)), dim3(256), 0, ctx->stream, d_u, d_v, n, cnt, off, ctx->sg_threshold, single, slot_v,
+                           slot_u, ctx->sg_key.as<int32_t>());
+        s.so = single_row_args(ctx, which, cnt);
         s.slot_v = slot_v; s.slot_u = slot_u;
         s.stage = ctx->sg_rows.as<float>(); s.stage_b = ctx->sg_bias.as<float>();
         const float scale = hub_scale(!s.is_d, n);
@@ -1388,13 +1499,15 @@
         slot = ctx->sgp_slot.as<int32_t>();
     } else {
         hipLaunchKernelGGL(path_count_kernel, pgrid, dim3(256), 0, ctx->stream, p.paths, p.path_len, p.stride, p.n_walks, cnt, slot, (const unsigned long long *)nullptr);
-        rc = device_segment_rows(ctx, cnt, ctx->n_node, ctx->sg_threshold, off, ctx->sg_list.as<int4>(), ctx->sg_tot.as<int64_t>());
+        const bool single = single_rows_on(ctx);
+        rc = device_segment_rows(ctx, cnt, ctx->n_node, single ? 2 : 1, ctx->sg_threshold, off, ctx->sg_list.as<int4>(), ctx->sg_tot.as<int64_t>());
         if (rc != GG_OK) return rc;
         rc = hub_index(ctx, cnt, off, ctx->sg_hub, ctx->sg_tot.as<int64_t>(), ctx->stream);
         if (rc != GG_OK) return rc;
-        hipLaunchKernelGGL(path_slot_kernel, pgrid, dim3(256), 0, ctx->stream, p.paths, p.path_len, p.stride, p.n_walks, cnt, off, ctx->sg_threshold, slot,
-                           ctx->sg_key.as<int32_t>(), (const unsigned long long *)nullptr);
-    }
+        hipLaunchKernelGGL(path_slot_kernel, pgrid, dim3(256), 0, ctx->stream, p.paths, p.path_len, p.stride, p.n_walks, cnt, off, ctx->sg_threshold, single,
+                           slot, ctx->sg_key.as<int32_t>(), (const unsigned long long *)nullptr);
+    }
+    p.so = single_row_args(ctx, 0, early ? ctx->sgp_cnt.as<int32_t>() : cnt);
     p.slot = slot;
     p.stage = ctx->sg_rows.as<float>();
     p.stage_b = ctx->sg_bias.as<float>();
@@ -1433,12 +1546,13 @@
     const dim3 pgrid((unsigned)cdiv(n_pos, 256));
     int32_t *cnt = ctx->sgp_cnt.as<int32_t>(), *off = ctx->sgp_off.as<int32_t>(), *slot = ctx->sgp_slot.as<int32_t>();
     hipLaunchKernelGGL(path_count_kernel, pgrid, dim3(256), 0, st, ctx->w_paths.as<int32_t>(), ctx->w_len.as<int32_t>(), ctx->w_stride, n_walks, cnt, slot, flag);
-    int rc = device_segment_rows(ctx, cnt, ctx->n_node, ctx->sg_threshold, off, ctx->sgp_list.as<int4>(), ctx->sgp_tot.as<int64_t>(), st, &ctx->sgp_scan);
+    const bool single = single_rows_on(ctx);
+    int rc = device_segment_rows(ctx, cnt, ctx->n_node, single ? 2 : 1, ctx->sg_threshold, off, ctx->sgp_list.as<int4>(), ctx->sgp_tot.as<int64_t>(), st, &ctx->sgp_scan);
     if (rc != GG_OK) return rc;
     rc = hub_index(ctx, cnt, off, ctx->sgp_hub, ctx->sgp_tot.as<int64_t>(), st);
     if (rc != GG_OK) return rc;
     hipLaunchKernelGGL(path_slot_kernel, pgrid, dim3(256), 0, st, ctx->w_paths.as<int32_t>(), ctx->w_len.as<int32_t>(), ctx->w_stride, n_walks, cnt, off,
-                       ctx->sg_threshold, slot, ctx->sgp_key.as<int32_t>(), flag);
+                       ctx->sg_threshold, single, slot, ctx->sgp_key.as<int32_t>(), flag);
     GG_HIP(ctx, hipGetLastError());
     GG_HIP(ctx, hipEventRecord(ctx->ev_slots_done, st));
     ctx->g_slots_ready = true;
diff --git a/graphgan_amd/engine.py b/graphgan_amd/engine.py
--- a/graphgan_amd/engine.py
+++ b/graphgan_amd/engine.py
@@ -579,6 +579,12 @@
     def load_state(self, path):
         self._ck(lib.gg_load_state(self._ctx, path.encode()))
 
+    def stage_stats(self, which):
+        self.synchronize()
+        out = np.zeros(5, dtype=np.uint64)
+        self._ck(lib.gg_debug_words(self._ctx, 1600 + 8 * int(which), 5, _ptr(out)))
+        return dict(zip(("reduced_rows", "stage_rows", "hub_rows", "single_rows", "passes"), (int(x) for x in out)))
+
     def counters(self):
         c = GGCounters()
         self._ck(lib.gg_get_counters(self._ctx, ctypes.byref(c)))
```

Result: slower. 602.0 million (-5.0%).
